# YangHai-1218/SCFlow

Hardware: AMD Instinct MI355X
Metric: image-pairs/sec at 256x256, 8 GRU iters (higher is better)
Workload: dtype f32

## Files before the change

include/scflow_hip.h:

```cpp
#ifndef SCFLOW_HIP_H
#define SCFLOW_HIP_H

#include <stdint.h>

#ifdef __cplusplus
extern "C" {
#endif

typedef void* scf_stream_t;

enum {
  SCF_OK = 0,
  SCF_EINVAL = -1,
  SCF_EUNSUPPORTED = -2,
  SCF_ELAUNCH = -3,
  SCF_ENODEVICE = -4
};

#define SCF_MAX_LEVELS 12

enum { SCF_ACT_NONE = 0, SCF_ACT_RELU = 1, SCF_ACT_SIGMOID = 2, SCF_ACT_TANH = 3 };

enum {
  SCF_CONV_PLAIN = 0,
  SCF_CONV_GRU_ZR = 1,
  SCF_CONV_GRU_Q = 2
};

#define SCF_ABI_MAJOR 5
#define SCF_VERSION (SCF_ABI_MAJOR * 100 + 3)
int scf_version(void);
const char* scf_error_string(int code);
int scf_device_count(void);

int scf_corr_build(const float* feat1, const float* feat2, float* const* levels,
                   int N, int C, int h, int w, int L, scf_stream_t stream);

int scf_corr_lookup(const float* const* levels, const float* flow, float* out,
                    int N, int h, int w, int r, int L, scf_stream_t stream);

int64_t scf_corr_level_floats(int h, int w, int level, int tiled);
unsigned scf_corr_preferred_layout(int h, int w, int r, int L);
int scf_corr_build_ex(const float* feat1, const float* feat2, float* const* levels, int N, int C,
                      int h, int w, int L, unsigned tiled_levels, scf_stream_t stream);
int scf_corr_lookup_ex(const float* const* levels, const float* flow, float* out, int N, int h,
                       int w, int r, int L, unsigned tiled_levels, scf_stream_t stream);

typedef struct scf_conv_desc {
  const float* in0; const float* in1;
  int32_t C0, C1;
  int64_t in0_nstride, in1_nstride;
  int32_t N, H, W;
  const float* wp;
  int64_t w_nstride;
  int32_t Mld;
  int32_t Cout;
  int32_t KH, KW, stride, pad_h, pad_w;
  int32_t KC;
  float* out; int64_t out_nstride;
  const float* bias;
  const float* scale; const float* shift;
  const float* res; int64_t res_nstride;
  float out_div;
  int32_t act, act2, act_split;
  int32_t mode;
  const float* gru_h; int64_t gru_h_nstride;
  float* gru_aux; int64_t gru_aux_nstride;
  const float* gru_z; int64_t gru_z_nstride;
  const void* wp_f16;
  const float* wp_a4;
  int32_t a4_groups;
  int32_t a4_mld;
  const float* wp_a4s;
  int32_t a4s_groups;
  const float* wp_thin;
  int32_t out_tile8x4;
  const float* wp_taps;
  const float* wp_a4t;
  int32_t a4t_groups;
  const float* wp_wino1d;
  const float* wp_wino;
  const float* wp_wino1d4;
  int32_t k_slices;
  int64_t out_slice_stride;
} scf_conv_desc;

int scf_conv2d(const scf_conv_desc* desc, scf_stream_t stream);

int scf_conv_workspace(scf_stream_t stream, float* ptr, int64_t floats);

int scf_conv2d_pair(const scf_conv_desc* a, const scf_conv_desc* b, scf_stream_t stream);

int64_t scf_pack_conv_weight_size(int Cout, int Cin, int KH, int KW, int KC);
int scf_pack_conv_weight(const float* w, int Cout, int Cin, int KH, int KW, int KC, float* out);
int64_t scf_pack_conv_weight_a4_size(int Cout, int Cin, int KH, int KW, int groups);
int scf_pack_conv_weight_a4(const float* w, int Cout, int Cin, int KH, int KW, int groups, float* out);
int64_t scf_pack_conv_weight_taps_size(int Cout, int Cin, int KH, int KW);
int scf_pack_conv_weight_taps(const float* w, int Cout, int Cin, int KH, int KW, float* out);
int64_t scf_pack_conv_weight_wino1d_size(int32_t Cout, int32_t Cin);
int scf_pack_conv_weight_wino1d(const float* w, int32_t Cout, int32_t Cin, float* out);
int64_t scf_pack_conv_weight_wino1d4_size(int32_t Cout, int32_t Cin);
int scf_pack_conv_weight_wino1d4(const float* w, int32_t Cout, int32_t Cin, float* out);
int64_t scf_pack_conv_weight_wino_size(int32_t Cout, int32_t Cin);
int scf_pack_conv_weight_wino(const float* w, int32_t Cout, int32_t Cin, float* out);

typedef struct scf_gru_pass {
  int32_t KH, KW, pad_h, pad_w;
  const float* wp_zr; const float* bias_zr;
  const float* wp_q; const float* bias_q;
  const float* wp_zr_a4; const float* wp_q_a4; int32_t a4_groups;
  const void* wp_zr_f16; const void* wp_q_f16;
  const float* wp_zr_k32; const float* wp_q_k32;
  const float* wp_zr_a4s; const float* wp_q_a4s; int32_t a4s_groups;
  const float* wp_zr_a4t; const float* wp_q_a4t; int32_t a4t_groups;
  const float* wp_zr_wino1d; const float* wp_q_wino1d;
  const float* wp_zr_wino1d4; const float* wp_q_wino1d4;
} scf_gru_pass;

int scf_sepconv_gru(float* hx, int64_t hx_nstride, int N, int Ch, int Cx, int H, int W,
                    const scf_gru_pass* passes, int npass, float* z, float* rh,
                    scf_stream_t stream);

int scf_sepconv_gru_ctx(float* hx, int64_t hx_nstride, int N, int Ch, int Cc, int Cx, int H, int W,
                        const scf_gru_pass* passes, int npass, const float* const* ctx,
                        int64_t ctx_nstride, float* z, float* rh, scf_stream_t stream);

typedef struct scf_iter_gn {
  const float* gamma; const float* beta; float* out;
  int32_t C, HW, G; float eps;
} scf_iter_gn;

typedef struct scf_scflow_iter {
  int32_t struct_size;
  int32_t N, H, W, h, w;
  int32_t L, radius; uint32_t tiled_levels; int32_t corr_channels;
  const float* levels[SCF_MAX_LEVELS];
  float* flow_lr;
  float* corr;
  int32_t mask_flow, mask_corr;
  const float* mask_prev;
  float* flow_masked;
  scf_conv_desc flow0, flow1, corr0, corr1, outn;
  float* flow_copy_dst;
  float* hx; int64_t hx_nstride; int32_t Ch, Cc, Cx, npass;
  scf_gru_pass gru[2];
  const float* ctx[2]; int64_t ctx_nstride;
  float* z; float* rh;
  scf_conv_desc heads, fpred, mpred, menc0, menc1, denc0, denc1;
  scf_conv_desc pose[3];
  scf_iter_gn gn[3];
  const float* fc1_w; const float* fc1_b; float* fc1_out; int32_t fc1_K, fc1_O;
  const float* fc2_w; const float* fc2_b; float* fc2_out; int32_t fc2_O;
  int32_t fc_fused, fc1_slices, fc2_slices;
  const float* rot_w; const float* rot_b; float* rot_all; int32_t rot_O;
  const float* trans_w; const float* trans_b; float* trans_all; int32_t trans_O;
  const int64_t* label; int32_t num_class, label_mode;
  const float* depth; const float* K; const float* R0; const float* t0; float invalid_flow_num;
  const float* flow_in;
  const float* R_in; const float* t_in;
  float* flow_out; float* flow_pred; float* mask_up;
  float* R_out; float* t_out; float* d_rot; float* d_trans;
  scf_stream_t side_stream; int32_t overlap_flow, overlap_mask, overlap_up;
  void* lookup_timer;
} scf_scflow_iter;

int scf_scflow_iteration(const scf_scflow_iter* iter, scf_stream_t stream);

int scf_instance_norm(const float* x, const float* res, float* out, int64_t planes,
                      int HW, float eps, int relu, scf_stream_t stream);

int scf_group_norm_relu(const float* x, const float* gamma, const float* beta, float* out,
                        int N, int C, int HW, int G, float eps, scf_stream_t stream);
int scf_group_norm_relu_parts(const float* x, int parts, int64_t part_stride, const float* gamma,
                              const float* beta, float* out, int N, int C, int HW, int G, float eps,
                              scf_stream_t stream);

int scf_linear(const float* x, const float* W, const float* b, float* y, int N, int K,
               int O, int act, scf_stream_t stream);

int scf_linear_pair(const float* x, const float* W1, const float* b1, float* y1, int O1,
                    const float* W2, const float* b2, float* y2, int O2, int N, int K, int act,
                    scf_stream_t stream);

typedef struct scf_fc_desc {
  const float* x; int32_t x_parts; int64_t x_part_stride;
  const float* x_bias; int32_t x_relu;
  int32_t gn_groups, gn_hw; const float* gn_gamma; const float* gn_beta; float gn_eps;
  int32_t N, K;
  const float* W; const float* bias; float* y; int32_t O;
  const float* W2; const float* bias2; float* y2; int32_t O2;
  int32_t act;
  int32_t slices;
} scf_fc_desc;
int scf_fc_splitk(const scf_fc_desc* desc, scf_stream_t stream);

#define SCF_POSE_LABEL_PER_SAMPLE 1
#define SCF_POSE_DEPTH_LINEAR 2
int scf_pose_update(const float* rot_all, const float* trans_all, const int64_t* label,
                    int num_class, int label_mode, const float* R_in, const float* t_in,
                    float* d_rot, float* d_trans, float* R_out, float* t_out, int N,
                    scf_stream_t stream);

int scf_reproject_flow(const float* depth, const float* K, const float* R0, const float* t0,
                       const float* R, const float* t, float* flow, int N, int H, int W,
                       float invalid_num, scf_stream_t stream);

int scf_pose_error(const double* verts, int nv, const double* gt_r, const double* gt_t,
                   const double* pred_r, const double* pred_t, const double* K,
                   const int* sample_idx, int nsel, int symmetric, double* err3d, double* err2d,
                   scf_stream_t stream);

int scf_flow_corr_2d3d(const float* flow, const float* depth, const float* occ, float occ_thresh,
                       const float* K, const float* R0, const float* t0, int N, int H, int W,
                       float* pts2d, float* pts3d, float* conf, int32_t* count, scf_stream_t stream);

enum { SCF_PNP_SAMPLE_ALL = 0, SCF_PNP_SAMPLE_TOPK = 1, SCF_PNP_SAMPLE_RANDOM = 2 };
typedef struct scf_pnp_params {
  int32_t iterations;
  float reproj_error;
  int32_t sample_mode;
  int32_t sample_num;
  uint64_t seed;
} scf_pnp_params;
int64_t scf_pnp_workspace_bytes(int N, int capacity, const scf_pnp_params* params);
int scf_pnp_ransac(const float* pts2d, const float* pts3d, const float* conf, const int32_t* count, int N,
                   int capacity, const float* K, const float* R_ref, const float* t_ref,
                   const scf_pnp_params* params, float* R, float* t, int32_t* ok, int32_t* inliers,
                   void* workspace, scf_stream_t stream);

typedef struct scf_mesh_store {
  const float* verts;
  const float* normals;
  const float* colors;
  const int32_t* faces;
  const int32_t* vert_offset;
  const int32_t* face_offset;
  int32_t num_classes;
  int32_t max_faces;
} scf_mesh_store;
typedef struct scf_render_params {
  int32_t H, W;
  int32_t default_lights;
  int32_t seperate_lights;
  float background[3];
  float norm_mean[3];
  float norm_std[3];
} scf_render_params;
double scf_render_pixel_coord(int index, int size, int other);
int64_t scf_render_workspace_bytes(int N, int max_faces);
int scf_render_mesh(const scf_mesh_store* mesh, const int32_t* labels, const float* R, const float* t,
                    const float* K, int N, const scf_render_params* params, float* zbuf, int32_t* pix_to_face,
                    float* rgba, float* rgb_nchw, void* workspace, scf_stream_t stream);

typedef struct scf_patch_params {
  double aspect_ratio;
  double size_ratio;
  double min_expand;
  int32_t out_h, out_w;
  int32_t resize;
  int32_t vertex_stride;
  int32_t keep_ratio;
  int32_t clip_border;
  int32_t fix_clip_border_quirk;
  int32_t center;
  int32_t to_rgb;
  int32_t crop_pad_val[3];
  int32_t pad_val[3];
  float mean[3];
  float std[3];
} scf_patch_params;
int64_t scf_patch_workspace_bytes(int N);
int scf_patch_boxes(const scf_mesh_store* mesh, const int32_t* labels, const float* R, const float* t,
                    const float* K, const int32_t* crop_in, int N, int frame_h, int frame_w,
                    const scf_patch_params* params, float* box, int32_t* crop, float* scale, float* transform_matrix,
                    float* k, int32_t* valid, void* workspace, scf_stream_t stream);
int scf_patch_extract(const uint8_t* frames, int F, int frame_h, int frame_w, const int32_t* frame_index, int N,
                      const void* workspace, const scf_patch_params* params, float* out, scf_stream_t stream);

int scf_filter_flow_by_mask(float* flow, const float* mask, int N, int H, int W,
                            float invalid_num, int align_corners, scf_stream_t stream);

int64_t scf_cal_epe_workspace_bytes(int N, int H, int W);
int scf_cal_epe(const float* flow_tgt, const float* flow_pred, const float* mask, int N, int H, int W,
                float max_flow, const float* threshs, int nthr, int fix_threshold_quirk, float* err_map,
                float* mean, float* ratios, float* total_mean, float* total_ratios, void* workspace,
                scf_stream_t stream);

int scf_unproject_depth(const float* depth, const float* K, const float* R0, const float* t0,
// ... 22 lines not shown
```

include/scflow_hip_prof.h:

```cpp
#ifndef SCFLOW_HIP_PROF_H
#define SCFLOW_HIP_PROF_H

#include "scflow_hip.h"

#ifdef __cplusplus
extern "C" {
#endif

typedef void* scf_timer_t;
int scf_timer_create(scf_timer_t* timer);
int scf_timer_destroy(scf_timer_t timer);
int scf_timer_elapsed_us(scf_timer_t timer, float* microseconds);
int scf_timer_arm(scf_timer_t timer);

int scf_conv2d_query(const scf_conv_desc* desc, int32_t* info);

enum {
  SCF_KERNEL_THIN = 1,
  SCF_KERNEL_TAPS = 2,
  SCF_KERNEL_WINO = 3,
  SCF_KERNEL_WINO1D = 4,
  SCF_KERNEL_F16X3 = 5,
  SCF_KERNEL_DMA = 6,
  SCF_KERNEL_MFMA = 7,
  SCF_KERNEL_MFMA_KSPLIT = 8,
  SCF_KERNEL_WINO_Q = 9,
  SCF_KERNEL_WINO1D4 = 10
};
typedef struct scf_conv_log_entry {
  int32_t kernel;
  int32_t Cin, Cout, KH, KW, stride, Ho, Wo, N;
  int32_t mode;
  int32_t paired;
  int32_t variant;
} scf_conv_log_entry;
int scf_conv_log_enable(int capacity);
enum {
  SCF_TUNE_WINO_VARIANT = 1,
  SCF_TUNE_DMA_FORCE_KSPLIT = 2,
  SCF_TUNE_DMA_KSPLIT_GROUPS = 3,
  SCF_TUNE_WINO1D4 = 4,
  SCF_TUNE_CONV_AUTOSLICE = 7,
  SCF_TUNE_LOOKUP_STORE = 6,
  SCF_TUNE_ITER_MERGE = 8,
  SCF_TUNE_WINO1D4_HALF = 9,
  SCF_TUNE_CONV_PAIR = 10,
  SCF_TUNE_LOOKUP_PIPE = 5
};
int scf_tune(int key, int value);
int scf_conv_log_read(scf_conv_log_entry* out, int max_entries);

#ifdef __cplusplus
}
#endif
#endif
```

scflow_amd/_lib.py:

```python
from __future__ import annotations

import ctypes as C
import os

_HERE = os.path.dirname(os.path.abspath(__file__))
LIB_PATH = os.path.join(_HERE, 'csrc', 'libscflow_hip.so')

SCF_OK = 0
ACT_NONE, ACT_RELU, ACT_SIGMOID, ACT_TANH = 0, 1, 2, 3
CONV_PLAIN, CONV_GRU_ZR, CONV_GRU_Q = 0, 1, 2
MAX_LEVELS = 12
ABI_MAJOR = 5

_fp = C.c_void_p


class ConvDesc(C.Structure):
    _fields_ = [
        ('in0', _fp), ('in1', _fp),
        ('C0', C.c_int32), ('C1', C.c_int32),
        ('in0_nstride', C.c_int64), ('in1_nstride', C.c_int64),
        ('N', C.c_int32), ('H', C.c_int32), ('W', C.c_int32),
        ('wp', _fp), ('w_nstride', C.c_int64),
        ('Mld', C.c_int32), ('Cout', C.c_int32),
        ('KH', C.c_int32), ('KW', C.c_int32), ('stride', C.c_int32),
        ('pad_h', C.c_int32), ('pad_w', C.c_int32), ('KC', C.c_int32),
        ('out', _fp), ('out_nstride', C.c_int64),
        ('bias', _fp), ('scale', _fp), ('shift', _fp),
        ('res', _fp), ('res_nstride', C.c_int64),
        ('out_div', C.c_float),
        ('act', C.c_int32), ('act2', C.c_int32), ('act_split', C.c_int32),
        ('mode', C.c_int32),
        ('gru_h', _fp), ('gru_h_nstride', C.c_int64),
        ('gru_aux', _fp), ('gru_aux_nstride', C.c_int64),
        ('gru_z', _fp), ('gru_z_nstride', C.c_int64),
        ('wp_f16', _fp),
        ('wp_a4', _fp),
        ('a4_groups', C.c_int32),
        ('a4_mld', C.c_int32),
        ('wp_a4s', _fp),
        ('a4s_groups', C.c_int32),
        ('wp_thin', _fp),
        ('out_tile8x4', C.c_int32),
        ('wp_taps', _fp),
        ('wp_a4t', _fp),
        ('a4t_groups', C.c_int32),
        ('wp_wino1d', _fp),
        ('wp_wino', _fp),
        ('wp_wino1d4', _fp),
        ('k_slices', C.c_int32),
        ('out_slice_stride', C.c_int64),
    ]


class GruPass(C.Structure):
    _fields_ = [
        ('KH', C.c_int32), ('KW', C.c_int32), ('pad_h', C.c_int32), ('pad_w', C.c_int32),
        ('wp_zr', _fp), ('bias_zr', _fp), ('wp_q', _fp), ('bias_q', _fp),
        ('wp_zr_a4', _fp), ('wp_q_a4', _fp), ('a4_groups', C.c_int32),
        ('wp_zr_f16', _fp), ('wp_q_f16', _fp),
        ('wp_zr_k32', _fp), ('wp_q_k32', _fp),
        ('wp_zr_a4s', _fp), ('wp_q_a4s', _fp), ('a4s_groups', C.c_int32),
        ('wp_zr_a4t', _fp), ('wp_q_a4t', _fp), ('a4t_groups', C.c_int32),
        ('wp_zr_wino1d', _fp), ('wp_q_wino1d', _fp),
        ('wp_zr_wino1d4', _fp), ('wp_q_wino1d4', _fp),
    ]


class ConvLogEntry(C.Structure):
    _fields_ = [(n, C.c_int32) for n in ('kernel', 'Cin', 'Cout', 'KH', 'KW', 'stride', 'Ho', 'Wo', 'N', 'mode', 'paired', 'variant')]


KERNEL_NAMES = {1: 'thin', 2: 'taps', 3: 'winograd', 4: 'winograd F(2,5)', 5: 'f16x3', 6: 'direct-dma',
                7: 'direct-mfma', 8: 'direct-mfma-ksplit', 9: 'winograd-q', 10: 'winograd F(4,5)'}


class FcDesc(C.Structure):
    _fields_ = [('x', _fp), ('x_parts', C.c_int32), ('x_part_stride', C.c_int64),
                ('x_bias', _fp), ('x_relu', C.c_int32),
                ('gn_groups', C.c_int32), ('gn_hw', C.c_int32), ('gn_gamma', _fp), ('gn_beta', _fp), ('gn_eps', C.c_float),
                ('N', C.c_int32), ('K', C.c_int32),
                ('W', _fp), ('bias', _fp), ('y', _fp), ('O', C.c_int32),
                ('W2', _fp), ('bias2', _fp), ('y2', _fp), ('O2', C.c_int32),
                ('act', C.c_int32), ('slices', C.c_int32)]


class PnpParams(C.Structure):
    _fields_ = [('iterations', C.c_int32), ('reproj_error', C.c_float), ('sample_mode', C.c_int32),
                ('sample_num', C.c_int32), ('seed', C.c_uint64)]


PNP_SAMPLE_ALL, PNP_SAMPLE_TOPK, PNP_SAMPLE_RANDOM = 0, 1, 2


class MeshStore(C.Structure):
    _fields_ = [('verts', _fp), ('normals', _fp), ('colors', _fp), ('faces', _fp), ('vert_offset', _fp),
                ('face_offset', _fp), ('num_classes', C.c_int32), ('max_faces', C.c_int32)]


class RenderParams(C.Structure):
    _fields_ = [('H', C.c_int32), ('W', C.c_int32), ('default_lights', C.c_int32), ('seperate_lights', C.c_int32),
                ('background', C.c_float * 3), ('norm_mean', C.c_float * 3), ('norm_std', C.c_float * 3)]


class PatchParams(C.Structure):
    _fields_ = [('aspect_ratio', C.c_double), ('size_ratio', C.c_double), ('min_expand', C.c_double),
                ('out_h', C.c_int32), ('out_w', C.c_int32), ('resize', C.c_int32), ('vertex_stride', C.c_int32),
                ('keep_ratio', C.c_int32), ('clip_border', C.c_int32), ('fix_clip_border_quirk', C.c_int32),
                ('center', C.c_int32), ('to_rgb', C.c_int32), ('crop_pad_val', C.c_int32 * 3),
                ('pad_val', C.c_int32 * 3), ('mean', C.c_float * 3), ('std', C.c_float * 3)]


class IterGN(C.Structure):
    _fields_ = [('gamma', _fp), ('beta', _fp), ('out', _fp),
                ('C', C.c_int32), ('HW', C.c_int32), ('G', C.c_int32), ('eps', C.c_float)]


class ScflowIter(C.Structure):
    _fields_ = [
        ('struct_size', C.c_int32),
        ('N', C.c_int32), ('H', C.c_int32), ('W', C.c_int32), ('h', C.c_int32), ('w', C.c_int32),
        ('L', C.c_int32), ('radius', C.c_int32), ('tiled_levels', C.c_uint32), ('corr_channels', C.c_int32),
        ('levels', _fp * MAX_LEVELS),
        ('flow_lr', _fp), ('corr', _fp),
        ('mask_flow', C.c_int32), ('mask_corr', C.c_int32), ('mask_prev', _fp), ('flow_masked', _fp),
        ('flow0', ConvDesc), ('flow1', ConvDesc), ('corr0', ConvDesc), ('corr1', ConvDesc), ('outn', ConvDesc),
        ('flow_copy_dst', _fp),
        ('hx', _fp), ('hx_nstride', C.c_int64), ('Ch', C.c_int32), ('Cc', C.c_int32), ('Cx', C.c_int32),
        ('npass', C.c_int32),
        ('gru', GruPass * 2), ('ctx', _fp * 2), ('ctx_nstride', C.c_int64), ('z', _fp), ('rh', _fp),
        ('heads', ConvDesc), ('fpred', ConvDesc), ('mpred', ConvDesc), ('menc0', ConvDesc), ('menc1', ConvDesc),
        ('denc0', ConvDesc), ('denc1', ConvDesc),
        ('pose', ConvDesc * 3), ('gn', IterGN * 3),
        ('fc1_w', _fp), ('fc1_b', _fp), ('fc1_out', _fp), ('fc1_K', C.c_int32), ('fc1_O', C.c_int32),
        ('fc2_w', _fp), ('fc2_b', _fp), ('fc2_out', _fp), ('fc2_O', C.c_int32),
        ('fc_fused', C.c_int32), ('fc1_slices', C.c_int32), ('fc2_slices', C.c_int32),
        ('rot_w', _fp), ('rot_b', _fp), ('rot_all', _fp), ('rot_O', C.c_int32),
        ('trans_w', _fp), ('trans_b', _fp), ('trans_all', _fp), ('trans_O', C.c_int32),
        ('label', _fp), ('num_class', C.c_int32), ('label_mode', C.c_int32),
        ('depth', _fp), ('K', _fp), ('R0', _fp), ('t0', _fp), ('invalid_flow_num', C.c_float),
        ('flow_in', _fp), ('R_in', _fp), ('t_in', _fp),
        ('flow_out', _fp), ('flow_pred', _fp), ('mask_up', _fp),
        ('R_out', _fp), ('t_out', _fp), ('d_rot', _fp), ('d_trans', _fp),
        ('side_stream', _fp), ('overlap_flow', C.c_int32), ('overlap_mask', C.c_int32), ('overlap_up', C.c_int32),
        ('lookup_timer', _fp),
    ]


SIGNATURES = {
    'scf_version': (C.c_int, []),
    'scf_error_string': (C.c_char_p, [C.c_int]),
    'scf_device_count': (C.c_int, []),
    'scf_corr_build': (C.c_int, [_fp, _fp, C.POINTER(_fp), C.c_int, C.c_int, C.c_int, C.c_int,
                                 C.c_int, _fp]),
    'scf_corr_lookup': (C.c_int, [C.POINTER(_fp), _fp, _fp, C.c_int, C.c_int, C.c_int, C.c_int,
                                  C.c_int, _fp]),
    'scf_corr_build_ex': (C.c_int, [_fp, _fp, C.POINTER(_fp), C.c_int, C.c_int, C.c_int, C.c_int,
                                    C.c_int, C.c_uint, _fp]),
    'scf_corr_lookup_ex': (C.c_int, [C.POINTER(_fp), _fp, _fp, C.c_int, C.c_int, C.c_int, C.c_int,
                                     C.c_int, C.c_uint, _fp]),
    'scf_corr_level_floats': (C.c_int64, [C.c_int, C.c_int, C.c_int, C.c_int]),
    'scf_corr_preferred_layout': (C.c_uint, [C.c_int, C.c_int, C.c_int, C.c_int]),
    'scf_pose_error': (C.c_int, [_fp, C.c_int, _fp, _fp, _fp, _fp, _fp, _fp, C.c_int, C.c_int, _fp, _fp, _fp]),
    'scf_filter_flow_by_mask': (C.c_int, [_fp, _fp, C.c_int, C.c_int, C.c_int, C.c_float, C.c_int, _fp]),
    'scf_cal_epe_workspace_bytes': (C.c_int64, [C.c_int, C.c_int, C.c_int]),
    'scf_cal_epe': (C.c_int, [_fp, _fp, _fp, C.c_int, C.c_int, C.c_int, C.c_float, C.POINTER(C.c_float), C.c_int, C.c_int,
                              _fp, _fp, _fp, _fp, _fp, _fp, _fp]),
    'scf_timer_create': (C.c_int, [C.POINTER(_fp)]),
    'scf_timer_destroy': (C.c_int, [_fp]),
    'scf_timer_arm': (C.c_int, [_fp]),
    'scf_timer_elapsed_us': (C.c_int, [_fp, C.POINTER(C.c_float)]),
    'scf_conv2d': (C.c_int, [C.POINTER(ConvDesc), _fp]),
    'scf_conv2d_pair': (C.c_int, [C.POINTER(ConvDesc), C.POINTER(ConvDesc), _fp]),
    'scf_conv2d_query': (C.c_int, [C.POINTER(ConvDesc), C.POINTER(C.c_int32)]),
    'scf_tune': (C.c_int, [C.c_int, C.c_int]),
    'scf_conv_log_enable': (C.c_int, [C.c_int]),
    'scf_conv_log_read': (C.c_int, [C.POINTER(ConvLogEntry), C.c_int]),
    'scf_pack_conv_weight_size': (C.c_int64, [C.c_int, C.c_int, C.c_int, C.c_int, C.c_int]),
    'scf_pack_conv_weight': (C.c_int, [_fp, C.c_int, C.c_int, C.c_int, C.c_int, C.c_int, _fp]),
    'scf_pack_conv_weight_a4_size': (C.c_int64, [C.c_int, C.c_int, C.c_int, C.c_int, C.c_int]),
    'scf_pack_conv_weight_a4': (C.c_int, [_fp, C.c_int, C.c_int, C.c_int, C.c_int, C.c_int, _fp]),
    'scf_pack_conv_weight_taps_size': (C.c_int64, [C.c_int, C.c_int, C.c_int, C.c_int]),
    'scf_pack_conv_weight_taps': (C.c_int, [_fp, C.c_int, C.c_int, C.c_int, C.c_int, _fp]),
    'scf_pack_conv_weight_wino1d_size': (C.c_int64, [C.c_int32, C.c_int32]),
    'scf_pack_conv_weight_wino1d': (C.c_int, [_fp, C.c_int32, C.c_int32, _fp]),
    'scf_pack_conv_weight_wino1d4_size': (C.c_int64, [C.c_int32, C.c_int32]),
    'scf_pack_conv_weight_wino1d4': (C.c_int, [_fp, C.c_int32, C.c_int32, _fp]),
    'scf_pack_conv_weight_wino_size': (C.c_int64, [C.c_int32, C.c_int32]),
    'scf_pack_conv_weight_wino': (C.c_int, [_fp, C.c_int32, C.c_int32, _fp]),
    'scf_sepconv_gru': (C.c_int, [_fp, C.c_int64, C.c_int, C.c_int, C.c_int, C.c_int, C.c_int,
                                  C.POINTER(GruPass), C.c_int, _fp, _fp, _fp]),
    'scf_sepconv_gru_ctx': (C.c_int, [_fp, C.c_int64, C.c_int, C.c_int, C.c_int, C.c_int, C.c_int,
                                      C.c_int, C.POINTER(GruPass), C.c_int, C.POINTER(_fp),
                                      C.c_int64, _fp, _fp, _fp]),
    'scf_scflow_iteration': (C.c_int, [C.POINTER(ScflowIter), _fp]),
    'scf_instance_norm': (C.c_int, [_fp, _fp, _fp, C.c_int64, C.c_int, C.c_float, C.c_int, _fp]),
    'scf_group_norm_relu': (C.c_int, [_fp, _fp, _fp, _fp, C.c_int, C.c_int, C.c_int, C.c_int,
                                      C.c_float, _fp]),
    'scf_conv_workspace': (C.c_int, [_fp, _fp, C.c_int64]),
    'scf_group_norm_relu_parts': (C.c_int, [_fp, C.c_int, C.c_int64, _fp, _fp, _fp, C.c_int, C.c_int, C.c_int, C.c_int,
                                            C.c_float, _fp]),
    'scf_fc_splitk': (C.c_int, [C.POINTER(FcDesc), _fp]),
    'scf_linear': (C.c_int, [_fp, _fp, _fp, _fp, C.c_int, C.c_int, C.c_int, C.c_int, _fp]),
    'scf_linear_pair': (C.c_int, [_fp, _fp, _fp, _fp, C.c_int, _fp, _fp, _fp, C.c_int, C.c_int, C.c_int,
                                  C.c_int, _fp]),
    'scf_pose_update': (C.c_int, [_fp, _fp, _fp, C.c_int, C.c_int, _fp, _fp, _fp, _fp, _fp, _fp,
                                  C.c_int, _fp]),
    'scf_reproject_flow': (C.c_int, [_fp, _fp, _fp, _fp, _fp, _fp, _fp, C.c_int, C.c_int,
                                     C.c_int, C.c_float, _fp]),
    'scf_flow_corr_2d3d': (C.c_int, [_fp, _fp, _fp, C.c_float, _fp, _fp, _fp, C.c_int, C.c_int, C.c_int,
                                     _fp, _fp, _fp, _fp, _fp]),
    'scf_pnp_workspace_bytes': (C.c_int64, [C.c_int, C.c_int, C.POINTER(PnpParams)]),
    'scf_pnp_ransac': (C.c_int, [_fp, _fp, _fp, _fp, C.c_int, C.c_int, _fp, _fp, _fp, C.POINTER(PnpParams),
                                 _fp, _fp, _fp, _fp, _fp, _fp]),
    'scf_render_pixel_coord': (C.c_double, [C.c_int, C.c_int, C.c_int]),
    'scf_render_workspace_bytes': (C.c_int64, [C.c_int, C.c_int]),
    'scf_render_mesh': (C.c_int, [C.POINTER(MeshStore), _fp, _fp, _fp, _fp, C.c_int, C.POINTER(RenderParams),
                                  _fp, _fp, _fp, _fp, _fp, _fp]),
    'scf_patch_workspace_bytes': (C.c_int64, [C.c_int]),
    'scf_patch_boxes': (C.c_int, [C.POINTER(MeshStore), _fp, _fp, _fp, _fp, _fp, C.c_int, C.c_int, C.c_int,
                                  C.POINTER(PatchParams), _fp, _fp, _fp, _fp, _fp, _fp, _fp, _fp]),
    'scf_patch_extract': (C.c_int, [_fp, C.c_int, C.c_int, C.c_int, _fp, C.c_int, _fp, C.POINTER(PatchParams), _fp,
                                    _fp]),
    'scf_unproject_depth': (C.c_int, [_fp, _fp, _fp, _fp, _fp, C.c_int, C.c_int, C.c_int, _fp]),
    'scf_resize_bilinear': (C.c_int, [_fp, _fp, _fp, C.c_int64, C.c_int, C.c_int, C.c_int,
                                      C.c_int, C.c_float, _fp]),
    'scf_convex_upsample': (C.c_int, [_fp, _fp, _fp, C.c_int, C.c_int, C.c_int, C.c_int, C.c_int,
                                      C.c_float, C.c_float, _fp]),
    'scf_avgpool2x2': (C.c_int, [_fp, _fp, C.c_int64, C.c_int, C.c_int, _fp]),
    'scf_mul_mask': (C.c_int, [_fp, C.c_int64, _fp, _fp, C.c_int64, C.c_int, C.c_int, C.c_int, _fp]),
    'scf_copy_strided': (C.c_int, [_fp, C.c_int64, _fp, C.c_int64, C.c_int, C.c_int64, _fp]),
}

_lib = None


class ScflowHipError(RuntimeError):
    pass


def load() -> C.CDLL:
    global _lib
    if _lib is not None:
        return _lib
    if not os.path.exists(LIB_PATH):
        raise ScflowHipError(
            f'{LIB_PATH} is missing: the HIP kernels are the product and there is no fallback. '
            'Build it with `python scflow_amd/csrc/build.py` (hipcc --offload-arch=gfx950).')
    lib = C.CDLL(LIB_PATH)
    lib.scf_version.restype = C.c_int
    have = lib.scf_version()
    if have // 100 != ABI_MAJOR:
        raise ScflowHipError(f'{LIB_PATH} was built with ABI major {have // 100}, this binding expects '
                             f'{ABI_MAJOR}: rebuild it (python scflow_amd/csrc/build.py --force)')
    for name, (res, args) in SIGNATURES.items():
        fn = getattr(lib, name)
        fn.restype = res
        fn.argtypes = args
    _lib = lib
    return lib


def check(code: int, what: str) -> None:
    if code != SCF_OK:
        msg = load().scf_error_string(code).decode()
        raise ScflowHipError(f'{what} failed: {msg} ({code})')
```

scflow_amd/csrc/conv_mfma.hip:

```cpp
#include <atomic>
#include <mutex>
#include <vector>
#include "scf_common.h"

typedef float f32x16 __attribute__((ext_vector_type(16)));
typedef float f32x4 __attribute__((ext_vector_type(4)));

#include "conv_kernels.h"

template <int WM, int WN, int NCP>
__device__ __forceinline__ void mfma_taps(f32x16 (&acc)[WM][WN], const float* wl, const float* pl,
                                          const int (&boff)[WN], int T, int KW, int KC, int BM,
                                          int PW, int PHW, int half, int l32) {
  for (int t = 0; t < T; ++t) {
    const int ky = t / KW, kx = t - ky * KW;
    const float* wt = wl + (t * KC + half) * BM + l32;
    const float* pt = pl + ky * PW + kx;
#pragma unroll
    for (int c = 0; c < NCP; ++c) {
      const int cp = 2 * c;
      float a[WM], b[WN];
#pragma unroll
      for (int i = 0; i < WM; ++i) a[i] = wt[cp * BM + i * 32];
#pragma unroll
// ... 508 lines not shown
  const ConvK& k = pl.k;
  const int N = d->N;
  const bool dry = r.info || r.cap;
  int32_t scratch[4];
  int32_t* info = r.info ? r.info : r.cap ? scratch : nullptr;
  hipStream_t st = scf_stream(stream);
  int out = SCF_EUNSUPPORTED;
  auto took = [&](int which, int rf) { r.which = which; out = rf; return rf != SCF_EUNSUPPORTED; };
  if (d->k_slices > 1) {
    r.which = SCF_KERNEL_DMA;
    return want_dma(d) ? scf_conv_dma_dispatch(k, N, dry, info, st, r.cap) : SCF_EUNSUPPORTED;
  }
  if (took(SCF_KERNEL_THIN, scf_conv_thin_dispatch(k, N, dry, st, r.cap))) return out;
  if (d->wp_taps && took(SCF_KERNEL_TAPS, scf_conv_taps_dispatch(k, d->wp_taps, N, dry, info, st, r.cap))) return out;
  if (d->wp_wino) {
    int quarter = 0;
    const int rw = scf_conv_wino_dispatch(k, d->wp_wino, N, dry, info, st, &quarter, r.cap);
    if (took(quarter ? SCF_KERNEL_WINO_Q : SCF_KERNEL_WINO, rw)) return out;
  }
  const int w4 = g_wino1d4.load(std::memory_order_relaxed);
  if (d->wp_wino1d4 && w4 && took(SCF_KERNEL_WINO1D4, scf_conv_wino1d4_dispatch(k, d->wp_wino1d4, N, w4 == 2, dry, info, st)))
    return out;
  if (d->wp_wino1d && took(SCF_KERNEL_WINO1D, scf_conv_wino1d_dispatch(k, d->wp_wino1d, N, dry, info, st))) return out;
  if (want_f16x3(d) && took(SCF_KERNEL_F16X3, scf_conv_f16x3_dispatch(k, N, dry, info, st))) return out;
  if (want_dma(d)) {
    float* ws = nullptr;
    int64_t ws_floats = 0;
    const bool sliced = !r.info && g_autoslice.load(std::memory_order_relaxed) && kws_lookup(st, &ws, &ws_floats);
    if (sliced && !dry) {
      const int S = scf_conv_dma_autoslice(k, N);
      const int64_t per_slice = (int64_t)N * d->Cout * k.Ho * k.Wo;
      if (S > 1 && per_slice * S <= ws_floats) {
        ConvK part = k;
        part.out = ws; part.out_ns = (long long)d->Cout * k.Ho * k.Wo;
        part.bias = nullptr; part.scale = nullptr; part.shift = nullptr; part.res = nullptr; part.res_ns = 0;
        part.out_div = 1.f; part.out_div_pow2 = 1; part.act = SCF_ACT_NONE; part.act2 = SCF_ACT_NONE; part.act_split = 0;
        part.mode = SCF_CONV_PLAIN; part.gru_h = nullptr; part.gru_aux = nullptr; part.gru_z = nullptr;
        part.kslices = S; part.slice_ns = per_slice;
        r.which = SCF_KERNEL_DMA;
        const int rs = scf_conv_dma_dispatch(part, N, false, nullptr, st);
        if (rs == SCF_OK) return scf_conv_kcombine_launch(k, ws, S, per_slice, N, st);
        if (rs != SCF_EUNSUPPORTED) return rs;
      }
    }
    if (took(SCF_KERNEL_DMA, scf_conv_dma_dispatch(k, N, dry, info, st, r.cap))) {
      if (sliced && r.cap) r.cap->variant = -1;
      return out;
    }
  }
  r.which = k.ksplit ? SCF_KERNEL_MFMA_KSPLIT : SCF_KERNEL_MFMA;
  const int WM = pl.WM, WN = pl.WN;
  if (dry) {
    if (r.info) {
      r.info[0] = WM; r.info[1] = WN; r.info[2] = (int32_t)pl.nblk;
      r.info[3] = k.T * (k.KC / 2) * WM * WN / (k.ksplit ? 4 : 1);
    }
    return SCF_OK;
  }
  const int nblk = (int)pl.nblk;
  if (k.ksplit) {
    if (k.KC == 32) return launch_ksplit<32>(k, nblk, pl.lds_bytes, st);
    if (k.KC == 8) return launch_ksplit<8>(k, nblk, pl.lds_bytes, st);
    return launch_ksplit<2>(k, nblk, pl.lds_bytes, st);
  }
#define SCF_CASE(M, Nn) if (WM == M && WN == Nn) return launch_conv<M, Nn>(k, nblk, pl.lds_bytes, st);
  SCF_CASE(1, 1) SCF_CASE(1, 2) SCF_CASE(2, 1) SCF_CASE(2, 2)
  SCF_CASE(3, 1) SCF_CASE(4, 1)
#undef SCF_CASE
  return SCF_EUNSUPPORTED;
}

namespace {
std::mutex g_log_mu;
std::vector<scf_conv_log_entry> g_log;
std::atomic<int> g_log_cap{0};
}

int scf_wino_variant_set(int v);
int scf_dma_force_ksplit_set(int v);
int scf_dma_ksplit_groups_set(int v);
int scf_lookup_pipe_set(int v);
int scf_lookup_store_set(int v);
int scf_iter_merge_set(int v);
int scf_wino1d4_half_set(int v);

extern "C" int scf_tune(int key, int value) {
  if (key == SCF_TUNE_WINO_VARIANT) return scf_wino_variant_set(value);
  if (key == SCF_TUNE_DMA_FORCE_KSPLIT) return scf_dma_force_ksplit_set(value);
  if (key == SCF_TUNE_DMA_KSPLIT_GROUPS) return scf_dma_ksplit_groups_set(value);
  if (key == SCF_TUNE_LOOKUP_PIPE) return scf_lookup_pipe_set(value);
  if (key == SCF_TUNE_LOOKUP_STORE) return scf_lookup_store_set(value);
  if (key == SCF_TUNE_ITER_MERGE) return scf_iter_merge_set(value);
  if (key == SCF_TUNE_WINO1D4_HALF) return scf_wino1d4_half_set(value);
  if (key == SCF_TUNE_CONV_AUTOSLICE) {
    if (value < 0 || value > 1) return SCF_EINVAL;
    return g_autoslice.exchange(value);
  }
  if (key == SCF_TUNE_CONV_PAIR) {
    if (value < 0 || value > 1) return SCF_EINVAL;
    return g_pair_mode.exchange(value);
  }
  if (key == SCF_TUNE_WINO1D4) {
    if (value < 0 || value > 2) return SCF_EINVAL;
    return g_wino1d4.exchange(value);
  }
  return SCF_EINVAL;
}

extern "C" int scf_conv_log_enable(int capacity) {
  std::lock_guard<std::mutex> lk(g_log_mu);
  g_log.clear();
  if (capacity > 0) g_log.reserve((size_t)capacity);
  else g_log.shrink_to_fit();
  g_log_cap.store(capacity > 0 ? capacity : 0);
  return SCF_OK;
}

extern "C" int scf_conv_log_read(scf_conv_log_entry* out, int max_entries) {
  std::lock_guard<std::mutex> lk(g_log_mu);
  const int n = (int)g_log.size();
  if (out)
    for (int i = 0; i < n && i < max_entries; ++i) out[i] = g_log[(size_t)i];
  return n;
}

static void conv_log_push(const scf_conv_desc* d, int which, int paired, int variant = -1);
extern "C" int scf_conv2d(const scf_conv_desc* d, scf_stream_t stream) {
  ConvReq r;
  const int rc = conv2d_walk(d, stream, r);
  if (rc == SCF_OK) conv_log_push(d, r.which, 0);
  return rc;
}

static void conv_log_push(const scf_conv_desc* d, int which, int paired, int variant) {
  if (g_log_cap.load(std::memory_order_relaxed) <= 0) return;
  std::lock_guard<std::mutex> lk(g_log_mu);
  if ((int)g_log.size() >= g_log_cap.load()) return;
  scf_conv_log_entry e;
  e.kernel = which; e.Cin = d->C0 + d->C1; e.Cout = d->Cout; e.KH = d->KH; e.KW = d->KW; e.stride = d->stride;
  e.Ho = (d->H + 2 * d->pad_h - d->KH) / d->stride + 1;
  e.Wo = (d->W + 2 * d->pad_w - d->KW) / d->stride + 1;
  e.N = d->N; e.mode = d->mode; e.paired = paired; e.variant = variant;
  g_log.push_back(e);
}

static bool pairable(int which, const ScfLaunchCap& c) {
  switch (which) {
    case SCF_KERNEL_THIN: return true;
    case SCF_KERNEL_TAPS: return c.variant >= 1;
    case SCF_KERNEL_WINO_Q: return c.variant >= 10 && c.variant < 20;
    case SCF_KERNEL_WINO: return c.variant >= 20;
    case SCF_KERNEL_DMA: return c.variant >= 0;
    default: return false;
  }
}

static bool capture(const scf_conv_desc* d, scf_stream_t stream, ScfLaunchCap* cap, int* which) {
  ConvReq r;
  r.cap = cap;
  const bool ok = conv2d_walk(d, stream, r) == SCF_OK && pairable(r.which, *cap);
  *which = r.which;
  return ok;
}

typedef int (*PairLaunch)(const ScfLaunchCap&, const ScfLaunchCap&, hipStream_t);

extern "C" int scf_conv2d_pair(const scf_conv_desc* a, const scf_conv_desc* b, scf_stream_t stream) {
  if (!a || !b) return SCF_EINVAL;
  ScfLaunchCap ca, cb;
  int fa = 0, fb = 0;
  if (g_pair_mode.load(std::memory_order_relaxed) != 1 && capture(a, stream, &ca, &fa) && capture(b, stream, &cb, &fb)) {
    const size_t lmax = ca.ldsb > cb.ldsb ? ca.ldsb : cb.ldsb;
    const long long slots = (long long)scf_cu_count() * (((fa == SCF_KERNEL_DMA || fb == SCF_KERNEL_DMA) && lmax > 80 * 1024) ? 1 : 2);
    const long long na = ca.nblk, nb = cb.nblk;
    auto rounds = [](long long n, long long s) { return (n + s - 1) / s; };
// ... 129 lines not shown
```

scflow_amd/csrc/norm.hip:

```cpp
#include "scf_common.h"

__device__ __forceinline__ float wave_sum(float v) {
#pragma unroll
  for (int off = 32; off > 0; off >>= 1) v += __shfl_xor(v, off);
  return v;
}

template <int NT>
__device__ __forceinline__ float block_sum(float v, float* red) {
  v = wave_sum(v);
  const int wave = threadIdx.x >> 6, lane = threadIdx.x & 63;
  __syncthreads();
  if (lane == 0) red[wave] = v;
  __syncthreads();
  float s = 0.f;
#pragma unroll
  for (int w = 0; w < NT / 64; w += 4) s += (red[w] + red[w + 1]) + (red[w + 2] + red[w + 3]);
  return s;
}

__device__ __forceinline__ float block_sum_256(float v, float* red) {
  v = wave_sum(v);
  const int wave = threadIdx.x >> 6, lane = threadIdx.x & 63;
  __syncthreads();
  if (lane == 0) red[wave] = v;
  __syncthreads();
  return (red[0] + red[1]) + (red[2] + red[3]);
}

template <int VEC4, int NT = 256>
__global__ __launch_bounds__(NT) void instance_norm_kernel(const float* x,
                                                           const float* res,
                                                           float* out, int HW,
                                                           float eps, int relu) {
  __shared__ float red[NT / 64];
  const long long pl = blockIdx.x;
  const float4* xp = reinterpret_cast<const float4*>(x + pl * HW);
  const int n4 = HW >> 2;
  float4 v[VEC4];
  float s = 0.f;
#pragma unroll
  for (int i = 0; i < VEC4; ++i) {
    const int idx = i * NT + threadIdx.x;
    v[i] = idx < n4 ? xp[idx] : make_float4(0.f, 0.f, 0.f, 0.f);
    s += (v[i].x + v[i].y) + (v[i].z + v[i].w);
  }
  const float mean = block_sum<NT>(s, red) / (float)HW;
  float q = 0.f;
#pragma unroll
  for (int i = 0; i < VEC4; ++i) {
    const int idx = i * NT + threadIdx.x;
    if (idx < n4) {
      const float a = v[i].x - mean, b = v[i].y - mean, c = v[i].z - mean, d = v[i].w - mean;
      q += (a * a + b * b) + (c * c + d * d);
    }
  }
  const float var = block_sum<NT>(q, red) / (float)HW;
  const float rstd = 1.0f / sqrtf(var + eps);
  float4* op = reinterpret_cast<float4*>(out + pl * HW);
  const float4* rp = res ? reinterpret_cast<const float4*>(res + pl * HW) : nullptr;
#pragma unroll
  for (int i = 0; i < VEC4; ++i) {
    const int idx = i * NT + threadIdx.x;
    if (idx < n4) {
      float4 o;
      o.x = (v[i].x - mean) * rstd;
      o.y = (v[i].y - mean) * rstd;
      o.z = (v[i].z - mean) * rstd;
      o.w = (v[i].w - mean) * rstd;
      if (rp) {
        const float4 r = rp[idx];
        o.x += r.x; o.y += r.y; o.z += r.z; o.w += r.w;
      }
      if (relu) {
        o.x = fmaxf(o.x, 0.f); o.y = fmaxf(o.y, 0.f); o.z = fmaxf(o.z, 0.f); o.w = fmaxf(o.w, 0.f);
      }
      scf_store4<(SCF_ST_SC1 & 2) != 0>(reinterpret_cast<float*>(op + idx), o.x, o.y, o.z, o.w);
    }
  }
}

__global__ __launch_bounds__(256) void instance_norm_generic_kernel(const float* x,
                                                                    const float* res,
                                                                    float* out, int HW,
                                                                    float eps, int relu) {
  __shared__ float red[4];
  const long long pl = blockIdx.x;
  const float* xp = x + pl * HW;
  float s = 0.f;
  for (int i = threadIdx.x; i < HW; i += 256) s += xp[i];
  const float mean = block_sum_256(s, red) / (float)HW;
  float q = 0.f;
  for (int i = threadIdx.x; i < HW; i += 256) {
    const float a = xp[i] - mean;
    q += a * a;
  }
  const float var = block_sum_256(q, red) / (float)HW;
  const float rstd = 1.0f / sqrtf(var + eps);
  for (int i = threadIdx.x; i < HW; i += 256) {
    float o = (xp[i] - mean) * rstd;
    if (res) o += res[pl * HW + i];
    if (relu) o = fmaxf(o, 0.f);
    out[pl * HW + i] = o;
  }
}

extern "C" int scf_instance_norm(const float* x, const float* res, float* out, int64_t planes,
                                 int HW, float eps, int relu, scf_stream_t stream) {
  if (!x || !out || planes <= 0 || HW <= 0) return SCF_EINVAL;
  if (planes > 0x7fffffffLL) return SCF_EUNSUPPORTED;
  hipStream_t st = scf_stream(stream);
  const dim3 grid((unsigned)planes), blk(256);
  const bool vec = (HW % 4 == 0) && ((((uintptr_t)x | (uintptr_t)out | (uintptr_t)res) & 15) == 0);
  const int n4 = HW / 4;
  if (vec && n4 <= 256) scf_launch(instance_norm_kernel<1>, grid, blk, 0, st, x, res, out, HW, eps, relu);
  else if (vec && n4 <= 1024) scf_launch(instance_norm_kernel<4>, grid, blk, 0, st, x, res, out, HW, eps, relu);
  else if (vec && n4 <= 4096) scf_launch(instance_norm_kernel<16>, grid, blk, 0, st, x, res, out, HW, eps, relu);
  else if (vec && n4 <= 8192) scf_launch((instance_norm_kernel<8, 1024>), grid, dim3(1024), 0, st, x, res, out, HW, eps, relu);
  else if (vec && n4 <= 20480) scf_launch((instance_norm_kernel<20, 1024>), grid, dim3(1024), 0, st, x, res, out, HW, eps, relu);
  else scf_launch(instance_norm_generic_kernel, grid, blk, 0, st, x, res, out, HW, eps, relu);
  return scf_launch_status();
}

__global__ __launch_bounds__(256) void group_norm_relu_kernel(const float* __restrict__ x, int parts,
                                                              long long part_stride,
                                                              const float* __restrict__ gamma,
                                                              const float* __restrict__ beta,
                                                              float* __restrict__ out, int C, int HW,
                                                              int G, float eps) {
  __shared__ float red[4];
  const int n = blockIdx.x / G, g = blockIdx.x % G;
  const int cpg = C / G;
  const int cnt = cpg * HW;
  const long long base = ((long long)n * C + (long long)g * cpg) * HW;
  const float* xp = x + base;
  auto at = [&](int i) {
    float v = xp[i];
    for (int sl = 1; sl < parts; ++sl) v += xp[(long long)sl * part_stride + i];
    return v;
  };
  constexpr int KEEP = 8;
  const bool keep = cnt <= KEEP * 256;
  float kv[KEEP];
  if (keep) {
    float u[4][KEEP];
#pragma unroll
    for (int j = 0; j < KEEP; ++j) {
      const int i = threadIdx.x + j * 256;
#pragma unroll
      for (int sl = 0; sl < 4; ++sl) u[sl][j] = (i < cnt && sl < parts) ? xp[(long long)sl * part_stride + i] : 0.f;
    }
#pragma unroll
    for (int j = 0; j < KEEP; ++j) {
      kv[j] = u[0][j];
#pragma unroll
      for (int sl = 1; sl < 4; ++sl)
        if (sl < parts) kv[j] += u[sl][j];
    }
    for (int sl = 4; sl < parts; ++sl) {
#pragma unroll
      for (int j = 0; j < KEEP; ++j) {
        const int i = threadIdx.x + j * 256;
        if (i < cnt) kv[j] += xp[(long long)sl * part_stride + i];
      }
    }
  }
  float s = 0.f;
  if (keep) {
#pragma unroll
    for (int j = 0; j < KEEP; ++j) s += kv[j];
  } else {
    for (int i = threadIdx.x; i < cnt; i += 256) s += at(i);
  }
  const float mean = block_sum_256(s, red) / (float)cnt;
  float q = 0.f;
  if (keep) {
#pragma unroll
    for (int j = 0; j < KEEP; ++j) {
      const float a = kv[j] - mean;
      q += (threadIdx.x + j * 256 < cnt) ? a * a : 0.f;
    }
  } else {
    for (int i = threadIdx.x; i < cnt; i += 256) {
      const float a = at(i) - mean;
      q += a * a;
    }
  }
  const float var = block_sum_256(q, red) / (float)cnt;
  const float rstd = 1.0f / sqrtf(var + eps);
  if (keep) {
#pragma unroll
    for (int j = 0; j < KEEP; ++j) {
      const int i = threadIdx.x + j * 256;
      if (i < cnt) {
        const int c = g * cpg + i / HW;
        out[base + i] = fmaxf((kv[j] - mean) * rstd * gamma[c] + beta[c], 0.f);
      }
    }
  } else {
    for (int i = threadIdx.x; i < cnt; i += 256) {
      const int c = g * cpg + i / HW;
      const float o = (at(i) - mean) * rstd * gamma[c] + beta[c];
      out[base + i] = fmaxf(o, 0.f);
// ... 102 lines not shown
```

scflow_amd/csrc/pose.hip:

```cpp
#include "scf_common.h"
#include "scf_pose.h"

struct PoseOut { float d_rot[6], d_trans[3], R[9], t[3]; };
struct PoseUpdateArgs {
  const float* rot_all; const float* trans_all; const long long* label; int num_class, label_mode;
  const float* R_in; const float* t_in; float* d_rot; float* d_trans; float* R_out; float* t_out;
};
__device__ __noinline__ void pose_update_one(const float* __restrict__ rot_all, const float* __restrict__ trans_all,
                                             const long long* __restrict__ label, int num_class, int label_mode,
                                             const float* R_in, const float* t_in, int n, PoseOut* o);
__device__ __forceinline__ void pose_store(const PoseOut& o, int n, float* __restrict__ d_rot, float* __restrict__ d_trans,
                                           float* R_out, float* t_out);

__global__ __launch_bounds__(256) void reproject_flow_kernel(
    const float* __restrict__ depth, const float* __restrict__ K, const float* __restrict__ R0,
    const float* __restrict__ t0, const float* R, const float* t,
    float* __restrict__ flow, int H, int W, float invalid, PoseUpdateArgs pu) {
  __shared__ PoseMats s;
  __shared__ PoseOut po;
  const int n = blockIdx.y;
  const bool fused = pu.rot_all != nullptr;
  if (fused && threadIdx.x == 224) {
    PoseOut o;
    pose_update_one(pu.rot_all, pu.trans_all, pu.label, pu.num_class, pu.label_mode, pu.R_in, pu.t_in, n, &o);
    po = o;
    if (blockIdx.x == 0) pose_store(o, n, pu.d_rot, pu.d_trans, pu.R_out, pu.t_out);
  }
  load_mats(&s, K, R0, t0, fused ? nullptr : R, fused ? nullptr : t, n);
  if (fused) {
    if (threadIdx.x < 9) s.R[threadIdx.x] = po.R[threadIdx.x];
    if (threadIdx.x >= 64 && threadIdx.x < 67) s.t[threadIdx.x - 64] = po.t[threadIdx.x - 64];
    __syncthreads();
  }
  const int hw = H * W;
  const float* dp = depth + (long long)n * hw;
  float* fx = flow + (long long)n * 2 * hw;
  float* fy = fx + hw;
  for (int idx = blockIdx.x * blockDim.x + threadIdx.x; idx < hw; idx += gridDim.x * blockDim.x) {
    const float d = dp[idx];
    float u = invalid, v = invalid;
    if (d > 0.f) {
      const int yi = idx / W, xi = idx - yi * W;
      const float x = (float)xi, y = (float)yi;
      float X, Y, Z;
      unproject(s, x, y, d, X, Y, Z);
      const float px = s.R[0] * X + s.R[1] * Y + s.R[2] * Z + s.t[0];
      const float py = s.R[3] * X + s.R[4] * Y + s.R[5] * Z + s.t[1];
      const float pz = s.R[6] * X + s.R[7] * Y + s.R[8] * Z + s.t[2];
      const float qx = s.K[0] * px + s.K[1] * py + s.K[2] * pz;
      const float qy = s.K[3] * px + s.K[4] * py + s.K[5] * pz;
      const float qz = s.K[6] * px + s.K[7] * py + s.K[8] * pz;
      u = qx / qz - x;
      v = qy / qz - y;
    }
    fx[idx] = u;
    fy[idx] = v;
  }
}

extern "C" int scf_reproject_flow(const float* depth, const float* K, const float* R0,
                                  const float* t0, const float* R, const float* t, float* flow,
                                  int N, int H, int W, float invalid_num, scf_stream_t stream) {
  if (!depth || !K || !R0 || !t0 || !R || !t || !flow || N <= 0 || H <= 0 || W <= 0) return SCF_EINVAL;
  if (N > 65535) return SCF_EUNSUPPORTED;
  const int bx = (int)(scf_cdiv((int64_t)H * W, 256) < 64 ? scf_cdiv((int64_t)H * W, 256) : 64);
  const PoseUpdateArgs none = {};
  scf_launch(reproject_flow_kernel, dim3(bx, N), dim3(256), 0, scf_stream(stream), depth, K,
                     R0, t0, R, t, flow, H, W, invalid_num, none);
  return scf_launch_status();
}

int scf_pose_update_reproject(const float* rot_all, const float* trans_all, const int64_t* label, int num_class,
                              int label_mode, const float* R_in, const float* t_in, float* d_rot, float* d_trans,
                              float* R_out, float* t_out, const float* depth, const float* K, const float* R0,
                              const float* t0, float* flow, int N, int H, int W, float invalid_num, scf_stream_t stream) {
  if (!rot_all || !trans_all || !label || !R_in || !t_in || !d_rot || !d_trans || !R_out || !t_out || num_class <= 0 ||
      (label_mode & ~(SCF_POSE_LABEL_PER_SAMPLE | SCF_POSE_DEPTH_LINEAR)))
    return SCF_EINVAL;
  if (!depth || !K || !R0 || !t0 || !flow || N <= 0 || H <= 0 || W <= 0) return SCF_EINVAL;
  if (N > 65535) return SCF_EUNSUPPORTED;
  if (R_in == R_out || t_in == t_out) return SCF_EUNSUPPORTED;
  int64_t cap = 2LL * scf_cu_count() / N;
  cap = cap < 64 ? 64 : cap;
  const int bx = (int)(scf_cdiv((int64_t)H * W, 256) < cap ? scf_cdiv((int64_t)H * W, 256) : cap);
  const PoseUpdateArgs pu = {rot_all, trans_all, (const long long*)label, num_class, label_mode, R_in, t_in,
                             d_rot, d_trans, R_out, t_out};
  scf_launch(reproject_flow_kernel, dim3(bx, N), dim3(256), 0, scf_stream(stream), depth, K,
                     R0, t0, (const float*)nullptr, (const float*)nullptr, flow, H, W, invalid_num, pu);
  return scf_launch_status();
}

__global__ __launch_bounds__(256) void unproject_depth_kernel(
    const float* __restrict__ depth, const float* __restrict__ K, const float* __restrict__ R0,
    const float* __restrict__ t0, float* __restrict__ pts, int H, int W) {
  __shared__ PoseMats s;
  const int n = blockIdx.y;
  load_mats(&s, K, R0, t0, nullptr, nullptr, n);
  const int hw = H * W;
  const float* dp = depth + (long long)n * hw;
  float* o = pts + (long long)n * 3 * hw;
  for (int idx = blockIdx.x * blockDim.x + threadIdx.x; idx < hw; idx += gridDim.x * blockDim.x) {
    const float d = dp[idx];
    float X = 0.f, Y = 0.f, Z = 0.f;
    if (d > 0.f) {
      const int yi = idx / W, xi = idx - yi * W;
      unproject(s, (float)xi, (float)yi, d, X, Y, Z);
    }
    o[idx] = X;
    o[hw + idx] = Y;
    o[2 * hw + idx] = Z;
  }
}

extern "C" int scf_unproject_depth(const float* depth, const float* K, const float* R0,
                                   const float* t0, float* pts, int N, int H, int W,
                                   scf_stream_t stream) {
  if (!depth || !K || !R0 || !t0 || !pts || N <= 0 || H <= 0 || W <= 0) return SCF_EINVAL;
  if (N > 65535) return SCF_EUNSUPPORTED;
  const int bx = (int)(scf_cdiv((int64_t)H * W, 256) < 64 ? scf_cdiv((int64_t)H * W, 256) : 64);
  scf_launch(unproject_depth_kernel, dim3(bx, N), dim3(256), 0, scf_stream(stream), depth,
                     K, R0, t0, pts, H, W);
  return scf_launch_status();
}

__device__ __noinline__ void pose_update_one(const float* __restrict__ rot_all, const float* __restrict__ trans_all,
                                             const long long* __restrict__ label, int num_class, int label_mode,
                                             const float* R_in, const float* t_in, int n, PoseOut* o) {
  long long cls = (label_mode & SCF_POSE_LABEL_PER_SAMPLE) ? label[n] : label[0];
  if (cls < 0) cls += num_class;
  if (cls < 0) cls = 0;
  if (cls >= num_class) cls = num_class - 1;
  const float* a = rot_all + ((long long)n * num_class + cls) * 6;
  const float* dt = trans_all + ((long long)n * num_class + cls) * 3;
  float o6[6], dtr[3];
  for (int i = 0; i < 6; ++i) { o6[i] = a[i]; o->d_rot[i] = o6[i]; }
  for (int i = 0; i < 3; ++i) { dtr[i] = dt[i]; o->d_trans[i] = dtr[i]; }
  float nx = sqrtf(o6[0] * o6[0] + o6[1] * o6[1] + o6[2] * o6[2]);
  nx = fmaxf(nx, 1e-12f);
  const float x0 = o6[0] / nx, x1 = o6[1] / nx, x2 = o6[2] / nx;
  float z0 = x1 * o6[5] - x2 * o6[4], z1 = x2 * o6[3] - x0 * o6[5], z2 = x0 * o6[4] - x1 * o6[3];
  float nz = fmaxf(sqrtf(z0 * z0 + z1 * z1 + z2 * z2), 1e-12f);
  z0 /= nz; z1 /= nz; z2 /= nz;
  const float y0 = z1 * x2 - z2 * x1, y1 = z2 * x0 - z0 * x2, y2 = z0 * x1 - z1 * x0;
  const float Rd[9] = {x0, y0, z0, x1, y1, z1, x2, y2, z2};
  float Rs[9], ts[3];
  for (int i = 0; i < 9; ++i) Rs[i] = R_in[n * 9 + i];
  for (int i = 0; i < 3; ++i) ts[i] = t_in[n * 3 + i];
  for (int r = 0; r < 3; ++r)
    for (int c = 0; c < 3; ++c)
      o->R[r * 3 + c] = Rd[r * 3 + 0] * Rs[0 * 3 + c] + Rd[r * 3 + 1] * Rs[1 * 3 + c] +
                        Rd[r * 3 + 2] * Rs[2 * 3 + c];
  const float vz = (label_mode & SCF_POSE_DEPTH_LINEAR) ? ts[2] * (dtr[2] + 1.f) : ts[2] / expf(dtr[2]);
  const float vx = vz * (dtr[0] / 10.f + ts[0] / ts[2]);
  const float vy = vz * (dtr[1] / 10.f + ts[1] / ts[2]);
  o->t[0] = vx;
  o->t[1] = vy;
  o->t[2] = vz;
}
__device__ __forceinline__ void pose_store(const PoseOut& o, int n, float* __restrict__ d_rot, float* __restrict__ d_trans,
                                           float* R_out, float* t_out) {
  for (int i = 0; i < 6; ++i) d_rot[n * 6 + i] = o.d_rot[i];
  for (int i = 0; i < 3; ++i) d_trans[n * 3 + i] = o.d_trans[i];
  for (int i = 0; i < 9; ++i) R_out[n * 9 + i] = o.R[i];
  for (int i = 0; i < 3; ++i) t_out[n * 3 + i] = o.t[i];
}

__global__ void pose_update_kernel(const float* __restrict__ rot_all,
                                   const float* __restrict__ trans_all,
                                   const long long* __restrict__ label, int num_class,
                                   int label_mode, const float* R_in, const float* t_in,
                                   float* __restrict__ d_rot, float* __restrict__ d_trans,
// ... 161 lines not shown
```

scflow_amd/csrc/scf_common.h:

```cpp
#pragma once
#include <hip/hip_runtime.h>
#include <hip/hip_ext.h>
#include <stdint.h>
#include <atomic>

#include "../../include/scflow_hip.h"
#include "../../include/scflow_hip_prof.h"

#define SCF_WAVE 64

static inline int scf_launch_status() {
  hipError_t e = hipGetLastError();
  return e == hipSuccess ? SCF_OK : SCF_ELAUNCH;
}

static inline hipStream_t scf_stream(scf_stream_t s) { return reinterpret_cast<hipStream_t>(s); }

static inline int64_t scf_cdiv(int64_t a, int64_t b) { return (a + b - 1) / b; }

static inline int scf_cu_count() {
  static int cus[64] = {0};
  int dev = 0;
  if (hipGetDevice(&dev) != hipSuccess || dev < 0 || dev >= 64) return 256;
  if (cus[dev] == 0) {
// ... 12 lines not shown
  if (hipFuncSetAttribute(fn, hipFuncAttributeMaxDynamicSharedMemorySize, bytes) != hipSuccess) return SCF_ELAUNCH;
  done.fetch_or(bit, std::memory_order_release);
  return SCF_OK;
}

struct ScfTimer { hipEvent_t start, stop; };
ScfTimer*& scf_armed_timer();

template <typename F, typename... Args>
static inline void scf_launch(F kernel, dim3 grid, dim3 block, size_t lds, hipStream_t st, Args... args) {
  ScfTimer*& slot = scf_armed_timer();
  if (slot) {
    ScfTimer* t = slot;
    slot = nullptr;
    hipExtLaunchKernelGGL(kernel, grid, block, (std::uint32_t)lds, st, t->start, t->stop, 0, args...);
  } else {
    hipLaunchKernelGGL(kernel, grid, block, lds, st, args...);
  }
}

__device__ __forceinline__ int scf_xcd_remap(int b, int nblk) {
  const int nx = 8;
  int q = nblk / nx, r = nblk % nx;
  int xcd = b % nx, slot = b / nx;
  int base = xcd < r ? xcd * (q + 1) : r * (q + 1) + (xcd - r) * q;
  return base + slot;
}

__device__ __forceinline__ float scf_fast_sigmoid(float v) {
  return __builtin_amdgcn_rcpf(1.f + __expf(-v));
}
__device__ __forceinline__ float scf_fast_tanh(float v) {
  const float t = __expf(-2.f * fabsf(v));
  const float r = (1.f - t) * __builtin_amdgcn_rcpf(1.f + t);
  return copysignf(r, v);
}

__device__ __forceinline__ float scf_apply_act(float v, int act) {
  switch (act) {
    case SCF_ACT_RELU: return v > 0.f ? v : 0.f;
    case SCF_ACT_SIGMOID: return 1.f / (1.f + expf(-v));
    case SCF_ACT_TANH: return tanhf(v);
    default: return v;
  }
}

#ifndef SCF_ST_SC1
#define SCF_ST_SC1 0
#endif
typedef float scf_st_f32x4 __attribute__((ext_vector_type(4)));
template <bool SC1>
__device__ __forceinline__ void scf_store4(float* p, float a, float b, float c, float d) {
  if constexpr (SC1) {
    const scf_st_f32x4 v = {a, b, c, d};
    asm volatile("global_store_dwordx4 %0, %1, off sc1\n\ts_nop 1" : : "v"(p), "v"(v) : "memory");
  } else {
    *reinterpret_cast<float4*>(p) = make_float4(a, b, c, d);
  }
}
typedef float scf_st_f32x2 __attribute__((ext_vector_type(2)));
template <bool SC1>
__device__ __forceinline__ void scf_store2(float* p, float a, float b) {
  if constexpr (SC1) {
    const scf_st_f32x2 v = {a, b};
    asm volatile("global_store_dwordx2 %0, %1, off sc1\n\ts_nop 1" : : "v"(p), "v"(v) : "memory");
  } else {
    *reinterpret_cast<scf_st_f32x2*>(p) = scf_st_f32x2{a, b};
  }
}
template <bool SC1>
__device__ __forceinline__ void scf_store1(float* p, float a) {
  if constexpr (SC1) asm volatile("global_store_dword %0, %1, off sc1" : : "v"(p), "v"(a) : "memory");
  else *p = a;
}

int scf_resize_bilinear_jobs(const float* a, const float* b, float* out, int64_t planes, float mul,
                             const float* a1, const float* b1, float* out1, int64_t planes1, float mul1,
                             float* out2, int out2_group, int64_t out2_gstride,
                             int Hin, int Win, int Hout, int Wout, scf_stream_t stream);
int scf_pose_update_reproject(const float* rot_all, const float* trans_all, const int64_t* label, int num_class,
                              int label_mode, const float* R_in, const float* t_in, float* d_rot, float* d_trans,
                              float* R_out, float* t_out, const float* depth, const float* K, const float* R0,
                              const float* t0, float* flow, int N, int H, int W, float invalid_num, scf_stream_t stream);
```

scflow_amd/csrc/scflow_iter.hip:

```cpp
#include "scf_common.h"

namespace {

struct IterEvents {
  hipEvent_t ev[7];
  bool ok = false;
  bool init() {
    if (ok) return true;
    for (int i = 0; i < 7; ++i)
      if (hipEventCreateWithFlags(&ev[i], hipEventDisableTiming) != hipSuccess) return false;
    return ok = true;
  }
};
IterEvents* iter_events() {
  static thread_local IterEvents pool[64];
  int dev = 0;
  if (hipGetDevice(&dev) != hipSuccess || dev < 0 || dev >= 64) return nullptr;
  return pool[dev].init() ? &pool[dev] : nullptr;
}

bool fork_to(hipStream_t from, hipStream_t to, hipEvent_t ev) {
  return hipEventRecord(ev, from) == hipSuccess && hipStreamWaitEvent(to, ev, 0) == hipSuccess;
}

struct OpenBranch {
  hipStream_t mainq, sideq;
  hipEvent_t join_ev;
  bool open = false;
  ~OpenBranch() {
    if (open) (void)fork_to(sideq, mainq, join_ev);
  }
};

#define SCF_TRY(call)                \
  do {                               \
    const int rc_ = (call);          \
    if (rc_ != SCF_OK) return rc_;   \
  } while (0)

}

static std::atomic<int> g_iter_merge{1};
int scf_iter_merge_set(int v) { return (v < 0 || v > 1) ? SCF_EINVAL : g_iter_merge.exchange(v); }

extern "C" int scf_scflow_iteration(const scf_scflow_iter* it, scf_stream_t stream) {
  if (!it) return SCF_EINVAL;
  const bool merge = g_iter_merge.load(std::memory_order_relaxed) != 0;
  if (it->struct_size != (int32_t)sizeof(scf_scflow_iter)) return SCF_EINVAL;
  if (!it->flow_in || !it->flow_out || !it->flow_pred || !it->mask_up || !it->flow_lr || !it->corr ||
      !it->R_in || !it->t_in || !it->R_out || !it->t_out || !it->d_rot || !it->d_trans || !it->hx ||
      it->N <= 0 || it->H <= 0 || it->W <= 0 || it->h <= 0 || it->w <= 0 || it->npass <= 0 || it->npass > 2)
    return SCF_EINVAL;
  if ((it->mask_flow || it->mask_corr) && !it->mask_prev) return SCF_EINVAL;
  const bool pair_flow = it->overlap_flow == 2, pair_mask = it->overlap_mask == 2;
  const bool any_overlap = it->overlap_flow == 1 || it->overlap_mask == 1 || it->overlap_up == 1;
  if (any_overlap && !it->side_stream) return SCF_EINVAL;
  hipStream_t mainq = scf_stream(stream), sideq = scf_stream(it->side_stream);
  IterEvents* Ep = any_overlap ? iter_events() : nullptr;
  if (any_overlap && !Ep) return SCF_ELAUNCH;
  static IterEvents none;
  IterEvents& E = Ep ? *Ep : none;
  OpenBranch br{mainq, sideq, E.ev[6]};
  const int N = it->N, hw = it->h * it->w;
  const float scale = (float)it->H / (float)it->h;

  const bool dual = merge && !it->mask_flow && it->flow_copy_dst != nullptr;
  SCF_TRY(scf_resize_bilinear_jobs(it->flow_in, nullptr, it->flow_lr, (int64_t)N * 2, 1.0f / scale, nullptr, nullptr, nullptr,
                                   0, 1.0f, dual ? it->flow_copy_dst : nullptr, 2, it->hx_nstride, it->H, it->W, it->h,
                                   it->w, stream));
  const float* flow_enc = it->flow_lr;
  if (it->mask_flow) {
    if (!it->flow_masked) return SCF_EINVAL;
    SCF_TRY(scf_mul_mask(it->flow_lr, (int64_t)2 * hw, it->mask_prev, it->flow_masked, (int64_t)2 * hw, N, 2, hw, stream));
    flow_enc = it->flow_masked;
  }
  if (it->overlap_flow == 1) {
    if (!fork_to(mainq, sideq, E.ev[0])) return SCF_ELAUNCH;
    br.open = true;
  }
  if (it->lookup_timer) scf_timer_arm(it->lookup_timer);
  const int rl = scf_corr_lookup_ex(it->levels, it->flow_lr, it->corr, N, it->h, it->w, it->radius, it->L,
                                    it->tiled_levels, stream);
  if (it->lookup_timer) scf_timer_arm(nullptr);
  SCF_TRY(rl);
  if (it->mask_corr)
    SCF_TRY(scf_mul_mask(it->corr, (int64_t)it->corr_channels * hw, it->mask_prev, it->corr,
                         (int64_t)it->corr_channels * hw, N, it->corr_channels, hw, stream));
  {
    scf_stream_t fq = it->overlap_flow == 1 ? it->side_stream : stream;
    scf_conv_desc f0 = it->flow0;
    f0.in0 = flow_enc;
    if (pair_flow) {
      SCF_TRY(scf_conv2d_pair(&it->corr0, &f0, stream));
      SCF_TRY(scf_conv2d_pair(&it->corr1, &it->flow1, stream));
    } else {
      SCF_TRY(scf_conv2d(&f0, fq));
      SCF_TRY(scf_conv2d(&it->flow1, fq));
      SCF_TRY(scf_conv2d(&it->corr0, stream));
      SCF_TRY(scf_conv2d(&it->corr1, stream));
    }
    if (it->overlap_flow == 1) {
      br.open = false;
      if (!fork_to(sideq, mainq, E.ev[1])) return SCF_ELAUNCH;
    }
    SCF_TRY(scf_conv2d(&it->outn, stream));
    if (!dual)
      SCF_TRY(scf_copy_strided(flow_enc, (int64_t)2 * hw, it->flow_copy_dst, it->hx_nstride, N, (int64_t)2 * hw, stream));
  }
  if (it->ctx[0])
    SCF_TRY(scf_sepconv_gru_ctx(it->hx, it->hx_nstride, N, it->Ch, it->Cc, it->Cx, it->h, it->w, it->gru, it->npass,
                                it->ctx, it->ctx_nstride, it->z, it->rh, stream));
  else
    SCF_TRY(scf_sepconv_gru(it->hx, it->hx_nstride, N, it->Ch, it->Cc + it->Cx, it->h, it->w, it->gru, it->npass,
                            it->z, it->rh, stream));
  SCF_TRY(scf_conv2d(&it->heads, stream));
  const bool mpred_aside = merge && it->overlap_mask == 1;
  if (mpred_aside) {
    if (!fork_to(mainq, sideq, E.ev[2])) return SCF_ELAUNCH;
    br.open = true;
  }
  if (pair_mask) {
    SCF_TRY(scf_conv2d_pair(&it->fpred, &it->mpred, stream));
  } else {
    SCF_TRY(scf_conv2d(&it->fpred, stream));
    if (!mpred_aside) SCF_TRY(scf_conv2d(&it->mpred, stream));
  }
  if (pair_mask) {
    SCF_TRY(scf_conv2d_pair(&it->denc0, &it->menc0, stream));
    SCF_TRY(scf_conv2d_pair(&it->denc1, &it->menc1, stream));
  } else {
    scf_stream_t mq = it->overlap_mask == 1 ? it->side_stream : stream;
    if (it->overlap_mask == 1 && !mpred_aside) {
      if (!fork_to(mainq, sideq, E.ev[2])) return SCF_ELAUNCH;
      br.open = true;
    }
    if (mpred_aside) SCF_TRY(scf_conv2d(&it->mpred, mq));
    SCF_TRY(scf_conv2d(&it->menc0, mq));
    SCF_TRY(scf_conv2d(&it->menc1, mq));
    SCF_TRY(scf_conv2d(&it->denc0, stream));
    SCF_TRY(scf_conv2d(&it->denc1, stream));
    if (it->overlap_mask == 1) {
      br.open = false;
      if (!fork_to(sideq, mainq, E.ev[3])) return SCF_ELAUNCH;
    }
  }
  {
    scf_stream_t uq = it->overlap_up == 1 ? it->side_stream : stream;
    if (it->overlap_up == 1) {
      if (!fork_to(mainq, sideq, E.ev[4])) return SCF_ELAUNCH;
      br.open = true;
    }
    if (!merge) {
      SCF_TRY(scf_resize_bilinear(it->flow_lr, it->fpred.out, it->flow_pred, (int64_t)N * 2, it->h, it->w, it->H, it->W,
                                  scale, uq));
      SCF_TRY(scf_resize_bilinear(it->mpred.out, nullptr, it->mask_up, (int64_t)N, it->h, it->w, it->H, it->W, 1.0f, uq));
    } else {
      SCF_TRY(scf_resize_bilinear_jobs(it->flow_lr, it->fpred.out, it->flow_pred, (int64_t)N * 2, scale, it->mpred.out, nullptr,
                                       it->mask_up, (int64_t)N, 1.0f, nullptr, 1, 0, it->h, it->w, it->H, it->W, uq));
    }
  }
  for (int i = 0; i < 3; ++i) {
    SCF_TRY(scf_conv2d(&it->pose[i], stream));
    const scf_iter_gn& g = it->gn[i];
    if (it->fc_fused && i == 2) break;
    const scf_conv_desc& pc = it->pose[i];
    SCF_TRY(scf_group_norm_relu_parts(pc.out, pc.k_slices > 1 ? pc.k_slices : 1, pc.out_slice_stride, g.gamma, g.beta, g.out,
                                      N, g.C, g.HW, g.G, g.eps, stream));
  }
  if (it->fc_fused) {
    const scf_iter_gn& g = it->gn[2];
    scf_fc_desc f = {};
    f.x = it->pose[2].out; f.x_parts = it->pose[2].k_slices > 1 ? it->pose[2].k_slices : 1;
    f.x_part_stride = it->pose[2].out_slice_stride; f.gn_groups = g.G; f.gn_hw = g.HW; f.gn_gamma = g.gamma; f.gn_beta = g.beta;
    f.gn_eps = g.eps; f.N = N; f.K = it->fc1_K; f.W = it->fc1_w; f.y = it->fc1_out; f.O = it->fc1_O; f.slices = it->fc1_slices;
    SCF_TRY(scf_fc_splitk(&f, stream));
    scf_fc_desc f2 = {};
    f2.x = it->fc1_out; f2.x_parts = it->fc1_slices; f2.x_part_stride = (int64_t)N * it->fc1_O; f2.x_bias = it->fc1_b;
    f2.x_relu = 1; f2.N = N; f2.K = it->fc1_O; f2.W = it->fc2_w; f2.y = it->fc2_out; f2.O = it->fc2_O; f2.slices = it->fc2_slices;
    SCF_TRY(scf_fc_splitk(&f2, stream));
    scf_fc_desc f3 = {};
    f3.x = it->fc2_out; f3.x_parts = it->fc2_slices; f3.x_part_stride = (int64_t)N * it->fc2_O; f3.x_bias = it->fc2_b;
    f3.x_relu = 1; f3.N = N; f3.K = it->fc2_O; f3.W = it->rot_w; f3.bias = it->rot_b; f3.y = it->rot_all; f3.O = it->rot_O;
    f3.W2 = it->trans_w; f3.bias2 = it->trans_b; f3.y2 = it->trans_all; f3.O2 = it->trans_O; f3.act = SCF_ACT_NONE; f3.slices = 1;
    SCF_TRY(scf_fc_splitk(&f3, stream));
  } else {
    SCF_TRY(scf_linear(it->gn[2].out, it->fc1_w, it->fc1_b, it->fc1_out, N, it->fc1_K, it->fc1_O, SCF_ACT_RELU, stream));
    SCF_TRY(scf_linear(it->fc1_out, it->fc2_w, it->fc2_b, it->fc2_out, N, it->fc1_O, it->fc2_O, SCF_ACT_RELU, stream));
    SCF_TRY(scf_linear_pair(it->fc2_out, it->rot_w, it->rot_b, it->rot_all, it->rot_O, it->trans_w, it->trans_b,
                            it->trans_all, it->trans_O, N, it->fc2_O, SCF_ACT_NONE, stream));
  }
  {
    const int rf = !merge ? SCF_EUNSUPPORTED : scf_pose_update_reproject(it->rot_all, it->trans_all, it->label, it->num_class, it->label_mode, it->R_in,
                                             it->t_in, it->d_rot, it->d_trans, it->R_out, it->t_out, it->depth, it->K, it->R0,
                                             it->t0, it->flow_out, N, it->H, it->W, it->invalid_flow_num, stream);
    if (rf == SCF_EUNSUPPORTED) {
      SCF_TRY(scf_pose_update(it->rot_all, it->trans_all, it->label, it->num_class, it->label_mode, it->R_in, it->t_in,
                              it->d_rot, it->d_trans, it->R_out, it->t_out, N, stream));
      SCF_TRY(scf_reproject_flow(it->depth, it->K, it->R0, it->t0, it->R_out, it->t_out, it->flow_out, N, it->H, it->W,
                                 it->invalid_flow_num, stream));
    } else {
      SCF_TRY(rf);
    }
  }
  if (it->overlap_up == 1) {
    br.open = false;
    if (!fork_to(sideq, mainq, E.ev[5])) return SCF_ELAUNCH;
  }
  return SCF_OK;
}
```

scflow_amd/modules.py:

```python
from __future__ import annotations

from typing import Dict, List, Optional, Sequence, Tuple, Union

import torch
import torch.nn as nn

from . import ops
from .ops import (ACT_NONE, ACT_RELU, ACT_SIGMOID, ACT_TANH, CONV_GRU_Q, CONV_GRU_ZR, PackedConv)
from .registry import DECODERS, ENCODERS, HEAD, build_head

Tensor = torch.Tensor

_ACTS = {None: ACT_NONE, 'ReLU': ACT_RELU, 'Sigmoid': ACT_SIGMOID, 'Tanh': ACT_TANH}


def _act_code(act_cfg: Optional[dict]) -> int:
    if act_cfg is None:
        return ACT_NONE
    kind = act_cfg.get('type')
    if kind not in _ACTS:
        raise NotImplementedError(f'activation {kind} has no HIP epilogue')
    return _ACTS[kind]


# ... 27 lines not shown
        out, stack = [], [self]
        while stack:
            m = stack.pop()
            out.append(m)
            for c in m._modules.values():
                if c is not None and not isinstance(c, HipModule):
                    stack.append(c)
        return out

    def _pack_sources(self):
        return [t for m in self._pack_modules() for d in (m._parameters, m._buffers)
                for t in d.values() if t is not None]

    def _pack_key(self):
        refs = self.__dict__.get('_pack_refs')
        if refs is None:
            if type(self)._pack_sources is not HipModule._pack_sources:
                return tuple((t.data_ptr(), t._version) for t in self._pack_sources())
            refs = self.__dict__['_pack_refs'] = [(d, n) for m in self._pack_modules()
                                                  for d in (m._parameters, m._buffers) for n in d]
        key = []
        for d, n in refs:
            t = d.get(n)
            if t is not None:
                key.append((t.data_ptr(), t._version))
        return tuple(key)

    @property
    def packed(self):
        d = self.__dict__
        key = self._pack_key()
        if d.get('_packed') is None or d.get('_packed_key') != key:
            with torch.no_grad():
                d['_packed'] = self._pack()
            d['_packed_key'] = key
        return d['_packed']


class ConvBlock(HipModule):

    def __init__(self, cin, cout, kernel_size, stride=1, padding=0, act_cfg=dict(type='ReLU'),
                 norm_cfg: Optional[dict] = None):
        super().__init__()
        self.conv = nn.Conv2d(cin, cout, kernel_size, stride=stride, padding=padding,
                              bias=norm_cfg is None)
        self.act = _act_code(act_cfg)
        self.groups = None
        if norm_cfg is not None:
            if norm_cfg.get('type') != 'GN':
                raise NotImplementedError('ConvBlock supports GN only (pose head)')
            self.groups = norm_cfg['num_groups']
            self.gn = nn.GroupNorm(self.groups, cout, eps=norm_cfg.get('eps', 1e-5))

    def _pack(self) -> PackedConv:
        c = self.conv
        return PackedConv.from_weight(c.weight, c.bias, stride=c.stride[0], padding=c.padding)

    def forward(self, x0: Tensor, x1: Optional[Tensor] = None, out: Optional[Tensor] = None) -> Tensor:
        if self.groups is None:
            return ops.conv2d(self.packed, x0, x1, out=out, act=self.act)
        if self.act != ACT_RELU:
            raise NotImplementedError('GN is fused with ReLU only')
        ks = ops.conv_kslices_for(self.packed, x0, x1)
        y = ops.conv2d(self.packed, x0, x1, kslices=ks)
        return ops.group_norm_relu(y, self.gn.weight, self.gn.bias, self.groups, self.gn.eps, out=out)


class _BasicBlock(HipModule):

    def __init__(self, inplanes, planes, stride, kind, downsample: bool):
        super().__init__()
        tag = 'in' if kind == 'IN' else 'bn'
        mk = (lambda c: nn.InstanceNorm2d(c)) if kind == 'IN' else (lambda c: nn.BatchNorm2d(c))
        self.kind, self.stride, self.tag = kind, stride, tag
        self.conv1 = nn.Conv2d(inplanes, planes, 3, stride=stride, padding=1, bias=True)
        setattr(self, tag + '1', mk(planes))
        self.conv2 = nn.Conv2d(planes, planes, 3, padding=1, bias=True)
        setattr(self, tag + '2', mk(planes))
        self.downsample = None
        if downsample:
            self.downsample = nn.Sequential(nn.Conv2d(inplanes, planes, 1, stride=stride, bias=True),
                                            mk(planes))

    def _bn(self, m):
        return (m.weight, m.bias, m.running_mean, m.running_var) if self.kind == 'BN' else None

    def _pack(self):
        n1, n2 = getattr(self, self.tag + '1'), getattr(self, self.tag + '2')
        eps = n1.eps
        p = dict(c1=PackedConv.from_weight(self.conv1.weight, self.conv1.bias, self.stride, 1,
                                           bn=self._bn(n1), eps=eps),
                 c2=PackedConv.from_weight(self.conv2.weight, self.conv2.bias, 1, 1,
                                           bn=self._bn(n2), eps=eps))
        if self.downsample is not None:
            ds = self.downsample[0]
            p['ds'] = PackedConv.from_weight(ds.weight, ds.bias, self.stride, 0,
                                             bn=self._bn(self.downsample[1]), eps=eps)
        return p

    def forward(self, x: Tensor) -> Tensor:
        p = self.packed
        if self.kind == 'BN':
            y = ops.conv2d(p['c1'], x, act=ACT_RELU)
            idt = ops.conv2d(p['ds'], x) if 'ds' in p else x
            return ops.conv2d(p['c2'], y, res=idt, act=ACT_RELU)
        y = ops.conv2d(p['c1'], x)
        ops.instance_norm(y, relu=True, out=y)
        y2 = ops.conv2d(p['c2'], y)
        if 'ds' in p:
            idt = ops.conv2d(p['ds'], x)
            ops.instance_norm(idt, out=idt)
        else:
            idt = x
        return ops.instance_norm(y2, res=idt, relu=True, out=y2)


@ENCODERS.register_module()
class RAFTEncoder(HipModule):

    def __init__(self, in_channels: int, out_channels: int, scale: float = 1 / 8,
                 net_type: str = 'Basic', norm_cfg: dict = dict(type='BN', requires_grad=True),
                 init_cfg=None, **unsupported) -> None:
        super().__init__()
        if net_type != 'Basic':
            raise NotImplementedError("only net_type='Basic' is built (SCFlow config)")
        bad = {k: v for k, v in unsupported.items()
               if v not in (None, False, -1) and k not in ('conv_cfg',)}
        if bad:
            raise NotImplementedError(f'RAFTEncoder options not built: {sorted(bad)}')
        kind = norm_cfg['type']
        if kind not in ('IN', 'BN', 'SyncBN'):
            raise NotImplementedError(f'norm {kind}')
        kind = 'IN' if kind == 'IN' else 'BN'
        self.kind, self.tag = kind, ('in' if kind == 'IN' else 'bn')
        self.in_channels, self.out_channels, self.scale = in_channels, out_channels, scale
        mk = (lambda c: nn.InstanceNorm2d(c)) if kind == 'IN' else (lambda c: nn.BatchNorm2d(c))
        self.stem_stride = 1 if scale == 1 / 4 else 2
        self.conv1 = nn.Conv2d(in_channels, 64, 7, stride=self.stem_stride, padding=3, bias=True)
        setattr(self, self.tag + '1', mk(64))
        inplanes = 64
        self.res_layers = []
        for i, (planes, stride) in enumerate(zip((64, 96, 128), (1, 2, 2)), start=1):
            layer = nn.Sequential(
                _BasicBlock(inplanes, planes, stride, kind, stride != 1 or inplanes != planes),
                _BasicBlock(planes, planes, 1, kind, False))
            self.add_module(f'res_layer{i}', layer)
            self.res_layers.append(f'res_layer{i}')
            inplanes = planes
        self.conv2 = nn.Conv2d(128, out_channels, 1)

    def _pack(self):
        n1 = getattr(self, self.tag + '1')
        bn = (n1.weight, n1.bias, n1.running_mean, n1.running_var) if self.kind == 'BN' else None
        return dict(stem=PackedConv.from_weight(self.conv1.weight, self.conv1.bias,
                                                self.stem_stride, 3, bn=bn, eps=n1.eps),
                    head=PackedConv.from_weight(self.conv2.weight, self.conv2.bias, 1, 0))

    def forward(self, x: Tensor, out: Optional[Tensor] = None, head_act: int = ACT_NONE,
                head_act2: int = ACT_NONE, head_split: int = 0) -> Tensor:
        p = self.packed
        if self.kind == 'BN':
            x = ops.conv2d(p['stem'], x, act=ACT_RELU)
        else:
            x = ops.conv2d(p['stem'], x)
            ops.instance_norm(x, relu=True, out=x)
        for name in self.res_layers:
            for blk in getattr(self, name):
                x = blk(x)
        return ops.conv2d(p['head'], x, out=out, act=head_act, act2=head_act2,
                          act_split=head_split)


def encoder_pair_supported(fe: 'RAFTEncoder', ce: 'RAFTEncoder') -> bool:
    return (fe.kind == 'IN' and ce.kind == 'BN' and fe.stem_stride == ce.stem_stride and fe.in_channels == ce.in_channels
            and fe.res_layers == ce.res_layers)


def raft_encoder_pair(fe: 'RAFTEncoder', xf: Tensor, ce: 'RAFTEncoder', xc: Tensor, out_c: Optional[Tensor] = None,
                      head_act: int = ACT_NONE, head_act2: int = ACT_NONE, head_split: int = 0) -> Tuple[Tensor, Tensor]:
    if not encoder_pair_supported(fe, ce):
        raise ValueError('raft_encoder_pair: (InstanceNorm feature encoder, BatchNorm context encoder) of one layer geometry')
    pf, pc = fe.packed, ce.packed
    yf, yc = ops.conv2d_pair((pf['stem'], xf), (pc['stem'], xc, dict(act=ACT_RELU)))
    ops.instance_norm(yf, relu=True, out=yf)
    for name in fe.res_layers:
        for bf, bc in zip(getattr(fe, name), getattr(ce, name)):
            qf, qc = bf.packed, bc.packed
            tf_, tc_ = ops.conv2d_pair((qf['c1'], yf), (qc['c1'], yc, dict(act=ACT_RELU)))
            ops.instance_norm(tf_, relu=True, out=tf_)
            if 'ds' in qf:
                if_, ic_ = ops.conv2d_pair((qf['ds'], yf), (qc['ds'], yc))
                ops.instance_norm(if_, out=if_)
            else:
                if_, ic_ = yf, yc
            uf_, yc = ops.conv2d_pair((qf['c2'], tf_), (qc['c2'], tc_, dict(res=ic_, act=ACT_RELU)))
            yf = ops.instance_norm(uf_, res=if_, relu=True, out=uf_)
    return ops.conv2d_pair((pf['head'], yf), (pc['head'], yc, dict(out=out_c, act=head_act, act2=head_act2,
                                                                  act_split=head_split)))


class CorrelationPyramid(HipModule):

    def __init__(self, num_levels: int = 4) -> None:
        super().__init__()
        self.num_levels = num_levels

    def forward(self, feat1: Tensor, feat2: Tensor, tiled_levels: int = 0) -> List[Tensor]:
        return ops.corr_build(feat1, feat2, self.num_levels, tiled_levels=tiled_levels)


class CorrLookup(HipModule):

    def __init__(self, radius: int = 4, mode: str = 'bilinear', padding_mode: str = 'zeros',
                 align_corners: bool = True) -> None:
        super().__init__()
        if mode != 'bilinear' or padding_mode != 'zeros' or not align_corners:
            raise NotImplementedError('HIP CorrLookup: bilinear / zeros / align_corners=True')
        self.r = radius

    def forward(self, corr_pyramid: Sequence[Tensor], flow: Tensor,
                tiled_levels: int = 0) -> Tensor:
        return ops.corr_lookup(corr_pyramid, flow, self.r, tiled_levels=tiled_levels)


def _pyramid_layout(feat: Tensor, radius: int, num_levels: int, allow: bool = True) -> int:
    return ops.pyramid_layout(feat.shape[-2], feat.shape[-1], radius, num_levels) if allow else 0


class MotionEncoder(HipModule):

    def __init__(self, num_levels: int = 4, radius: int = 4, net_type: str = 'Basic',
                 conv_cfg=None, norm_cfg=None, act_cfg=dict(type='ReLU')) -> None:
        super().__init__()
        if net_type not in ('Basic', 'Large') or norm_cfg is not None:
            raise NotImplementedError('MotionEncoder: Basic, no norm')
        cin = num_levels * (2 * radius + 1) ** 2
        self.corr_net = nn.Sequential(ConvBlock(cin, 256, 1, padding=0, act_cfg=act_cfg),
                                      ConvBlock(256, 192, 3, padding=1, act_cfg=act_cfg))
        self.flow_net = nn.Sequential(ConvBlock(2, 128, 7, padding=3, act_cfg=act_cfg),
                                      ConvBlock(128, 64, 3, padding=1, act_cfg=act_cfg))
        self.out_net = nn.Sequential(ConvBlock(256, 126, 3, padding=1, act_cfg=act_cfg))
        self.out_channels = [126]

    def forward(self, corr: Tensor, flow: Tensor, out: Optional[Tensor] = None,
                overlap: bool = False, cf: Optional[Tensor] = None, fork=None) -> Tensor:
        n, _, h, w = flow.shape
        dev = flow.device
        if out is None:
            out = torch.empty((n, 128, h, w), dtype=torch.float32, device=dev)
        if cf is None:
            if overlap:
                raise ValueError('overlap=True needs a cf buffer allocated before the fork point')
            cf = torch.empty((n, 256, h, w), dtype=torch.float32, device=dev)
        if not overlap and 'flow' in ops.PAIR_BRANCHES and ops._CONV_EVENTS is None:
            cn, fn = self.corr_net, self.flow_net
            c1, f1 = ops.conv2d_pair((cn[0].packed, corr, dict(act=cn[0].act)), (fn[0].packed, flow, dict(act=fn[0].act)))
            ops.conv2d_pair((cn[1].packed, c1, dict(out=cf[:, :192], act=cn[1].act)),
                            (fn[1].packed, f1, dict(out=cf[:, 192:], act=fn[1].act)))
            del c1, f1
        else:
            br = ops.side_stream(overlap, after=fork)
            with br:
                f1 = self.flow_net[0](flow)
                self.flow_net[1](f1, out=cf[:, 192:])
                del f1
            c1 = self.corr_net[0](corr)
            self.corr_net[1](c1, out=cf[:, :192])
            br.join()
        self.out_net[0](cf, out=out[:, :126])
        ops.copy_channels(flow, out[:, 126:128])
        return out


class ConvGRU(HipModule):
    _kernel = {'Conv': [3], 'SeqConv': [(1, 5), (5, 1)]}
    _padding = {'Conv': [1], 'SeqConv': [(0, 2), (2, 0)]}

    def __init__(self, h_channels: int, x_channels: int, net_type: str = 'SeqConv') -> None:
        super().__init__()
# ... 210 lines not shown
        a, b = self.flow_pred.layers[0].conv, self.mask_pred.layers[0].conv
        return PackedConv.from_weight(torch.cat([a.weight, b.weight], 0),
                                      torch.cat([a.bias, b.bias], 0), 1, 1)

    def forward(self, feat_render: Tensor, feat_real: Tensor, h_feat: Tensor, cxt_feat: Tensor,
                ref_rotation: Tensor, ref_translation: Tensor, depth: Tensor, internel_k: Tensor,
                label: Tensor, init_flow: Tensor, invalid_flow_num: float,
                _consume_state: bool = False):
        hc, cc = self.h_channels, self.cxt_channels
        n, H, W = depth.shape
        scale = 2 ** (self.num_levels - 1)
        h, w = H // scale, W // scale
        dev = depth.device
        f32 = dict(dtype=torch.float32, device=dev)

        tiled = _pyramid_layout(feat_render, self.radius, self.num_levels, self.tiled_pyramid)
        pyramid = self.corr_block(feat_render, feat_real, tiled_levels=tiled)
        hx = _as_gru_buffer(h_feat, cxt_feat, hc + cc + 128, _consume_state)
        rot, trans = ref_rotation.contiguous(), ref_translation.contiguous()
        rot0, trans0 = rot, trans
        flow = init_flow
        outs = ([], [], [], [], [], [], [])
        dm = torch.empty((n, 96, h, w), **f32)
        heads = torch.empty((n, 512, h, w), **f32)
        ctx = self.gru.context_terms(hx[:, hc:hc + cc]) if self.hoist_context else None
        ov_flow, ov_mask, ov_up = (ops.small_work(n, H, W, b) for b in ('flow', 'mask', 'upsample'))
        if self.c_iteration and ops._CONV_EVENTS is None:
            return self._forward_c(pyramid, tiled, hx, ctx, rot0, trans0, depth, internel_k, label, init_flow,
                                   invalid_flow_num, tuple(ops.branch_mode(n, H, W, b) for b in ('flow', 'mask', 'upsample')))
        mask = ops.constant((n, 1, h, w), 1.0, dev) if (self.mask_flow or self.mask_corr) else None
        cf = torch.empty((n, 256, h, w), **f32)
        zbuf = torch.empty((2, n, hc, h, w), **f32)
        for _ in range(self.iters):
            flow_lr = ops.resize_bilinear(flow, (h, w), mul=1.0 / scale)
            flow_in = ops.mul_mask(flow_lr, mask) if self.mask_flow else flow_lr
            fork = ops.fork_point() if ov_flow else None
            corr = self.corr_lookup(pyramid, flow_lr, tiled_levels=tiled)
            if self.mask_corr:
                ops.mul_mask(corr, mask, out=corr)
            self.encoder(corr, flow_in, out=hx[:, hc + cc:], overlap=ov_flow, cf=cf, fork=fork)
            hv = self.gru.forward_inplace(hx, ctx, cc, scratch=zbuf)
            ops.conv2d(self.packed, hv, out=heads, act=ACT_RELU)
            d_flow = self.flow_pred.predict(heads[:, :256])
            mask = self.mask_pred.predict(heads[:, 256:], act=ACT_SIGMOID)
            br = ops.side_stream(ov_mask)
            with br:
                m1 = self.mask_encoder[0](mask)
                self.mask_encoder[1](m1, out=dm[:, 64:])
                del m1
            d1 = self.delta_flow_encoder[0](d_flow)
            self.delta_flow_encoder[1](d1, out=dm[:, :64])
            br.join()
            flow_pred = torch.empty((n, 2, H, W), **f32)
            up_mask = torch.empty((n, 1, H, W), **f32)
            br = ops.side_stream(ov_up)
            with br:
                ops.resize_bilinear(flow_lr, (H, W), mul=float(scale), b=d_flow, out=flow_pred)
                ops.resize_bilinear(mask, (H, W), out=up_mask)
            rot_all, trans_all = self.pose_pred.features(hv, dm)
            d_rot, d_trans, rot, trans = ops.pose_update(
                rot_all, trans_all, label, self.pose_pred.num_class, rot, trans,
                self.pose_flags())
            flow = ops.reproject_flow(depth, internel_k, rot0, trans0, rot, trans,
                                      invalid_flow_num)
            br.join()
            for lst, v in zip(outs, (flow, flow_pred, rot, trans, up_mask, d_rot, d_trans)):
                lst.append(v)
        return outs


def _scflow_forward_c(self, pyramid, tiled, hx, ctx, rot0, trans0, depth, internel_k, label, init_flow,
                      invalid_flow_num, overlap):
    from ._lib import ScflowIter
    import ctypes as C
    hc, cc = self.h_channels, self.cxt_channels
    n, H, W = depth.shape
    scale = 2 ** (self.num_levels - 1)
    h, w = H // scale, W // scale
    f32 = dict(dtype=torch.float32, device=depth.device)
    iters = self.iters
    E = lambda *shape: torch.empty(shape, **f32)
    enc, ph = self.encoder, self.pose_pred
    kch = self.num_levels * (2 * self.radius + 1) ** 2
    flow_lr, flow_m, corr = E(n, 2, h, w), (E(n, 2, h, w) if self.mask_flow else None), E(n, kch, h, w)
    f1, c1, cf = E(n, 128, h, w), E(n, 256, h, w), E(n, 256, h, w)
    zbuf, heads, dm = E(2, n, hc, h, w), E(n, 512, h, w), E(n, 96, h, w)
    d_flow, mask, m1, d1 = E(n, 2, h, w), E(n, 1, h, w), E(n, 64, h, w), E(n, 128, h, w)
    ones = ops.constant((n, 1, h, w), 1.0, depth.device) if (self.mask_flow or self.mask_corr) else None
    hv, xm = hx[:, :hc], hx[:, hc + cc:]
    flows, fpreds, masks = E(iters, n, 2, H, W), E(iters, n, 2, H, W), E(iters, n, 1, H, W)
    rots, transs, drots, dtranss = E(iters, n, 3, 3), E(iters, n, 3), E(iters, n, 6), E(iters, n, 3)
    it = ScflowIter()
    it.struct_size = C.sizeof(ScflowIter)
    it.N, it.H, it.W, it.h, it.w = n, H, W, h, w
    it.L, it.radius, it.tiled_levels, it.corr_channels = len(pyramid), self.radius, int(tiled), kch
    for l, lv in enumerate(pyramid):
        it.levels[l] = lv.data_ptr()
    it.flow_lr, it.corr = flow_lr.data_ptr(), corr.data_ptr()
    it.mask_flow, it.mask_corr = int(self.mask_flow), int(self.mask_corr)
    it.flow_masked = None if flow_m is None else flow_m.data_ptr()
    keep = [pyramid, flow_lr, flow_m, corr, f1, c1, cf, zbuf, heads, dm, d_flow, mask, m1, d1, ones, hx, ctx]
    cd = lambda blk, *a, **k: ops.conv_desc(blk.packed, *a, act=blk.act, **k)[0]
    it.flow0 = cd(enc.flow_net[0], flow_lr, out=f1)
    it.flow1 = cd(enc.flow_net[1], f1, out=cf[:, 192:])
    it.corr0 = cd(enc.corr_net[0], corr, out=c1)
    it.corr1 = cd(enc.corr_net[1], c1, out=cf[:, :192])
    it.outn = cd(enc.out_net[0], cf, out=xm[:, :126])
    it.flow_copy_dst = xm[:, 126:128].data_ptr()
    it.hx, it.hx_nstride = hx.data_ptr(), hx.stride(0)
    it.Ch, it.Cc, it.Cx = hc, cc, hx.shape[1] - hc - cc
    if ctx is not None:
        packs = [(pk[1], pk[2]) for pk in self.gru._ctx_packs(cc)]
        for i, t in enumerate(ctx):
            it.ctx[i] = t.data_ptr()
        it.ctx_nstride = ctx[0].stride(0)
    else:
        packs = self.gru.packed
    arr = ops.gru_passes(packs)
    it.npass = len(packs)
    for i in range(len(packs)):
        it.gru[i] = arr[i]
    it.z, it.rh = zbuf[0].data_ptr(), zbuf[1].data_ptr()
    it.heads = ops.conv_desc(self.packed, hv, out=heads, act=ACT_RELU)[0]
    it.fpred = ops.conv_desc(self.flow_pred.packed, heads[:, :256], out=d_flow)[0]
    it.mpred = ops.conv_desc(self.mask_pred.packed, heads[:, 256:], out=mask, act=ACT_SIGMOID)[0]
    it.menc0 = cd(self.mask_encoder[0], mask, out=m1)
    it.menc1 = cd(self.mask_encoder[1], m1, out=dm[:, 64:])
    it.denc0 = cd(self.delta_flow_encoder[0], d_flow, out=d1)
    it.denc1 = cd(self.delta_flow_encoder[1], d1, out=dm[:, :64])
    x0, x1 = hv, dm
    for i, blk in enumerate(ph.conv_layers):
        if blk.groups is None or blk.act != ACT_RELU:
            raise NotImplementedError('pose head: conv + GroupNorm + ReLU blocks')
        ks = ops.conv_kslices_for(blk.packed, x0, x1)
        d_, y = ops.conv_desc(blk.packed, x0, x1, kslices=ks)
        g = torch.empty_like(y[0] if ks > 1 else y)
        it.pose[i] = d_
        it.gn[i].gamma, it.gn[i].beta, it.gn[i].out = blk.gn.weight.data_ptr(), blk.gn.bias.data_ptr(), g.data_ptr()
        it.gn[i].C, it.gn[i].HW, it.gn[i].G, it.gn[i].eps = y.shape[-3], y.shape[-2] * y.shape[-1], blk.groups, blk.gn.eps
        keep += [y, g]
        x0, x1 = g, None
    fc1, fc2 = ph.fc_layers[0][0], ph.fc_layers[1][0]
    if fc1.in_features != x0[0].numel():
        raise _lib_error(f'pose head expects {fc1.in_features} features, the maps give {x0[0].numel()}')
    s1, s2 = ph.fc_plan()
    it.fc_fused, it.fc1_slices, it.fc2_slices = int(s1 > 0), max(s1, 1), max(s2, 1)
    y1, y2 = E(max(s1, 1), n, fc1.out_features), E(max(s2, 1), n, fc2.out_features)
    ra, ta = E(n, ph.rotation_pred.out_features), E(n, ph.translation_pred.out_features)
    keep += [y1, y2, ra, ta]
    P = lambda t: None if t is None else t.data_ptr()
    it.fc1_w, it.fc1_b, it.fc1_out, it.fc1_K, it.fc1_O = P(fc1.weight), P(fc1.bias), y1.data_ptr(), fc1.in_features, fc1.out_features
    it.fc2_w, it.fc2_b, it.fc2_out, it.fc2_O = P(fc2.weight), P(fc2.bias), y2.data_ptr(), fc2.out_features
    it.rot_w, it.rot_b, it.rot_all, it.rot_O = P(ph.rotation_pred.weight), P(ph.rotation_pred.bias), ra.data_ptr(), ra.shape[1]
    it.trans_w, it.trans_b, it.trans_all, it.trans_O = (P(ph.translation_pred.weight), P(ph.translation_pred.bias),
                                                        ta.data_ptr(), ta.shape[1])
    if not label.is_cuda or label.dtype != torch.int64 or not label.is_contiguous():
        raise _lib_error('label must be a contiguous int64 GPU tensor')
    it.label, it.num_class, it.label_mode = label.data_ptr(), ph.num_class, self.pose_flags()
    for name, t in (('depth', depth), ('internel_k', internel_k), ('ref_rotation', rot0), ('ref_translation', trans0),
                    ('init_flow', init_flow)):
        ops._dense(t, name)
    it.depth, it.K, it.R0, it.t0 = depth.data_ptr(), internel_k.data_ptr(), rot0.data_ptr(), trans0.data_ptr()
    it.invalid_flow_num = float(invalid_flow_num)
    it.overlap_flow, it.overlap_mask, it.overlap_up = (int(b) for b in overlap)
    it.side_stream = ops.side_stream_handle() if any(int(b) == 1 for b in overlap) else None
    outs = ([], [], [], [], [], [], [])
    flow, rot, trans = init_flow, rot0, trans0
    for i in range(iters):
        it.flow_in, it.R_in, it.t_in = flow.data_ptr(), rot.data_ptr(), trans.data_ptr()
        it.mask_prev = None if ones is None else (ones if i == 0 else mask).data_ptr()
        flow, rot, trans = flows[i], rots[i], transs[i]
        it.flow_out, it.flow_pred, it.mask_up = flow.data_ptr(), fpreds[i].data_ptr(), masks[i].data_ptr()
        it.R_out, it.t_out, it.d_rot, it.d_trans = rot.data_ptr(), trans.data_ptr(), drots[i].data_ptr(), dtranss[i].data_ptr()
        ops.scflow_iteration(it)
        for lst, v in zip(outs, (flow, fpreds[i], rot, trans, masks[i], drots[i], dtranss[i])):
            lst.append(v)
    if any(overlap):
        pass
    del keep
    return outs


def _lib_error(msg):
    from ._lib import ScflowHipError
    return ScflowHipError(msg)


SCFlowDecoder._forward_c = _scflow_forward_c


class _RAFTDecoderBase(HipModule):
    _h_channels = {'Basic': 128, 'Small': 96}
    _cxt_channels = {'Basic': 128, 'Small': 64}

    def __init__(self, net_type: str, num_levels: int, radius: int, iters: int,
                 corr_lookup_cfg: dict = dict(type='CorrLookup', align_corners=True),
                 gru_type: str = 'SeqConv', feat_channels: Union[int, Sequence[int]] = 256,
                 mask_channels: int = 64, convex_unsample_flow: bool = True, conv_cfg=None,
                 norm_cfg=None, act_cfg=None) -> None:
        super().__init__()
        if net_type != 'Basic':
            raise NotImplementedError("RAFT decoders: net_type='Basic'")
        self.net_type, self.num_levels, self.radius, self.iters = net_type, num_levels, radius, iters
        self.h_channels = self._h_channels[net_type]
        self.cxt_channels = self._cxt_channels[net_type]
        self.mask_channels = mask_channels * (2 * radius + 1)
        self.corr_block = CorrelationPyramid(num_levels)
        cl = dict(corr_lookup_cfg)
        cl.pop('type', None)
        cl['radius'] = radius
        self.corr_lookup = CorrLookup(**cl)
        self.encoder = MotionEncoder(num_levels, radius, net_type, conv_cfg, norm_cfg, act_cfg)
        self.gru = ConvGRU(self.h_channels, 126 + 2 + self.cxt_channels, gru_type)
        self.flow_pred = XHead(self.h_channels, [256], 2, x='flow')
        self.mask_pred = XHead(self.h_channels, [256], self.mask_channels, x='mask')
        self.convex_upsample_flow = convex_unsample_flow
        self.tiled_pyramid = True
        self.hoist_context = True
        if self.mask_channels != 9 * (2 ** (num_levels - 1)) ** 2:
            raise NotImplementedError('convex up-sampling kernel: 9 x 8 x 8 mask (radius 4, 4 levels)')

    def _context(self, hx):
        hc, cc = self.h_channels, self.cxt_channels
        return self.gru.context_terms(hx[:, hc:hc + cc]) if self.hoist_context else None

    def _step(self, pyramid, flow, hx, tiled=0, ctx=None):
        hc, cc = self.h_channels, self.cxt_channels
        corr = self.corr_lookup(pyramid, flow, tiled_levels=tiled)
        self.encoder(corr, flow, out=hx[:, hc + cc:])
        hv = self.gru.forward_inplace(hx, ctx, cc)
        d_flow = self.flow_pred(hv)
        n, _, h, w = flow.shape
        return hv, ops.resize_bilinear(flow, (h, w), b=d_flow)

    def _upsample(self, x: Tensor, mask: Optional[Tensor], mul: float) -> Tensor:
        scale = 2 ** (self.num_levels - 1)
        n, c, h, w = x.shape
        if mask is None:
            return ops.resize_bilinear(x, (scale * h, scale * w), mul=mul)
        return ops.convex_upsample(x, mask, scale, x_mul=mul, mask_mul=0.25)


@DECODERS.register_module()
class RAFTDecoder(_RAFTDecoderBase):

    def forward(self, feat1: Tensor, feat2: Tensor, flow: Tensor, h_feat: Tensor,
                cxt_feat: Tensor, _consume_state: bool = False) -> List[Tensor]:
        tiled = _pyramid_layout(feat1, self.radius, self.num_levels, self.tiled_pyramid)
        pyramid = self.corr_block(feat1, feat2, tiled_levels=tiled)
        hx = _as_gru_buffer(h_feat, cxt_feat, self.h_channels + self.cxt_channels + 128,
                            _consume_state)
        scale = float(2 ** (self.num_levels - 1))
        flow = flow.contiguous()
        outs = []
        ctx = self._context(hx)
        for _ in range(self.iters):
            hv, flow = self._step(pyramid, flow, hx, tiled, ctx)
            mask = self.mask_pred(hv) if self.convex_upsample_flow else None
            outs.append(self._upsample(flow, mask, scale))
# ... 44 lines not shown
```

scflow_amd/ops.py:

```python
from __future__ import annotations

import ctypes as C
import os
import math
from dataclasses import dataclass
from typing import List, Optional, Sequence, Tuple

import torch

from . import _lib
from ._lib import (ACT_NONE, ACT_RELU, ACT_SIGMOID, ACT_TANH, CONV_GRU_Q, CONV_GRU_ZR,
                   CONV_PLAIN, ConvDesc)

Tensor = torch.Tensor

__all__ = ['record_conv_kernels', 'PackedConv', 'conv_desc', 'gru_passes', 'scflow_iteration', 'side_stream_handle', 'pyramid_layout', 'untile_level', 'level_storage_shape', 'sepconv_gru', 'pack_conv_weight', 'pack_conv_weight_f16x3', 'set_conv_precision', 'set_conv_winograd', 'get_conv_winograd', 'pack_conv_weight_wino', 'pack_conv_weight_wino1d', 'pack_conv_weight_wino1d4',
           'get_conv_precision', 'set_conv_kslices', 'conv_kslices', 'conv_kslices_for', 'constant', 'clear_constants', 'register_conv_workspace', 'choose_kc', 'conv2d', 'conv2d_pair', 'corr_build', 'corr_lookup',
           'instance_norm', 'group_norm_relu', 'linear', 'fc_splitk', 'fc_slices', 'pose_update', 'reproject_flow',
           'flow_corr_2d3d', 'pnp_params', 'pnp_ransac', 'pnp',
           'unproject_depth', 'linear_pair', 'resize_bilinear', 'convex_upsample', 'avgpool2x2', 'copy_channels',
           'ACT_NONE', 'ACT_RELU', 'ACT_SIGMOID', 'ACT_TANH', 'CONV_PLAIN', 'CONV_GRU_ZR',
           'CONV_GRU_Q']


_cur_dev = torch._C._cuda_getDevice
_raw_stream = torch._C._cuda_getCurrentRawStream


_KWS = {}
_KWS_FLOATS = 1 << 20


def register_conv_workspace(enable: bool = True) -> None:
    dev = _cur_dev()
    handle = _raw_stream(dev)
    if enable:
        ws = torch.empty((_KWS_FLOATS,), dtype=torch.float32, device=f'cuda:{dev}')
        _lib.check(_lib.load().scf_conv_workspace(handle, ws.data_ptr(), _KWS_FLOATS), 'scf_conv_workspace')
        _KWS[(dev, handle)] = ws
    elif _KWS.pop((dev, handle), None) is not None:
        _lib.check(_lib.load().scf_conv_workspace(handle, None, 0), 'scf_conv_workspace')


def _stream() -> int:
    return _raw_stream(_cur_dev())


def _dev(t: Tensor, name: str) -> None:
    if not isinstance(t, torch.Tensor) or not t.is_cuda:
        raise _lib.ScflowHipError(f'{name}: expected a tensor on the GPU (HIP path only, no CPU '
                                  'fallback)')
    if t.dtype != torch.float32:
        raise _lib.ScflowHipError(f'{name}: expected float32, got {t.dtype}')
    if t.device.index != _cur_dev():
        raise _lib.ScflowHipError(
            f'{name} lives on cuda:{t.device.index} but the current device is '
            f'cuda:{_cur_dev()}: wrap the call in torch.cuda.device(tensor.device)')


def _dense(t: Tensor, name: str) -> int:
    _dev(t, name)
    if not t.is_contiguous():
        raise _lib.ScflowHipError(f'{name}: expected a contiguous tensor')
    return t.data_ptr()


def _nchw(t: Tensor, name: str) -> Tuple[int, int, int, int, int, int]:
    _dev(t, name)
    if t.dim() != 4:
        raise _lib.ScflowHipError(f'{name}: expected 4-D NCHW')
    n, c, h, w = t.shape
    sn, sc, sh, sw = t.stride()
    ok = (sw == 1 or w == 1) and (sh == w or h == 1) and (sc == h * w or c == 1)
    if not ok:
        raise _lib.ScflowHipError(f'{name}: not a sample-strided NCHW view (strides {t.stride()})')
    if n == 1:
        sn = c * h * w
    return t.data_ptr(), n, c, h, w, sn


def _opt(t: Optional[Tensor], name: str) -> Optional[int]:
    return None if t is None else _dense(t, name)


_SIDE = {}


OVERLAP_BRANCHES = set()
OVERLAP_MAX_PIXELS = {'context': 4 * 256 * 256, 'flow': 4 * 256 * 256, 'mask': 4 * 256 * 256, 'upsample': 4 * 256 * 256}


PAIR_BRANCHES = {'context', 'flow', 'mask'}
PAIR_MAX_PIXELS = {'context': 4 * 256 * 256, 'flow': None, 'mask': None}


def branch_mode(n: int, h: int, w: int, branch: str) -> int:
    if branch in PAIR_BRANCHES:
        lim = PAIR_MAX_PIXELS.get(branch, 4 * 256 * 256)
        return 2 if lim is None or n * h * w <= lim else 0
    lim = OVERLAP_MAX_PIXELS.get(branch, 4 * 256 * 256)
    return 1 if n * h * w <= lim and branch in OVERLAP_BRANCHES else 0
# ... 501 lines not shown
            g.wp_zr_a4s, g.wp_q_a4s, g.a4s_groups = pzr.wp4s.data_ptr(), pq.wp4s.data_ptr(), pzr.g4s
        if pzr.wp4t is not None and pq.wp4t is not None and pzr.g4t == pq.g4t:
            g.wp_zr_a4t, g.wp_q_a4t, g.a4t_groups = pzr.wp4t.data_ptr(), pq.wp4t.data_ptr(), pzr.g4t
        if _CONV_WINOGRAD and not f16 and pzr.wwino1d is not None and pq.wwino1d is not None:
            g.wp_zr_wino1d, g.wp_q_wino1d = pzr.wwino1d.data_ptr(), pq.wwino1d.data_ptr()
            if pzr.wwino1d4 is not None and pq.wwino1d4 is not None:
                g.wp_zr_wino1d4, g.wp_q_wino1d4 = pzr.wwino1d4.data_ptr(), pq.wwino1d4.data_ptr()
    return arr


gru_passes = _gru_passes


def side_stream_handle() -> int:
    main = torch.cuda.current_stream()
    key = (torch.cuda.current_device(), main.cuda_stream)
    side = _SIDE.get(key)
    if side is None:
        side = _SIDE[key] = torch.cuda.Stream(device=key[0])
    return side.cuda_stream


def scflow_iteration(it: '_lib.ScflowIter') -> None:
    lib = _lib.load()
    it.lookup_timer = _LOOKUP_TIMERS.take() if _LOOKUP_TIMERS is not None else None
    _lib.check(lib.scf_scflow_iteration(C.byref(it), _stream()), 'scf_scflow_iteration')


def sepconv_gru(packs, hx: Tensor, h_channels: int, z: Tensor, rh: Tensor,
                ctx: Optional[Sequence[Tensor]] = None, ctx_channels: int = 0) -> None:
    hc = h_channels
    if ctx is not None and (ctx_channels <= 0 or len(ctx) != len(packs)):
        raise _lib.ScflowHipError('sepconv_gru: one context term per pass, ctx_channels > 0')
    if _CONV_EVENTS is not None:
        hv, xv = hx[:, :hc], hx[:, hc + ctx_channels:]
        for i, (pzr, pq) in enumerate(packs):
            if ctx is None:
                conv2d(pzr, hx, out=z, mode=CONV_GRU_ZR, gru_h=hv, gru_aux=rh)
                conv2d(pq, rh, xv, out=hv, mode=CONV_GRU_Q, gru_h=hv, gru_z=z)
            else:
                conv2d(pzr, hv, xv, out=z, mode=CONV_GRU_ZR, gru_h=hv, gru_aux=rh, res=ctx[i][:, :2 * hc])
                conv2d(pq, rh, xv, out=hv, mode=CONV_GRU_Q, gru_h=hv, gru_z=z, res=ctx[i][:, 2 * hc:])
        return
    p, n, c, h, w, sn = _nchw(hx, 'hx')
    arr = _gru_passes(packs)
    if ctx is None:
        _lib.check(_lib.load().scf_sepconv_gru(p, sn, n, hc, c - hc, h, w, arr, len(packs),
                                               _dense(z, 'z'), _dense(rh, 'rh'), _stream()),
                   'scf_sepconv_gru')
        return
    ptrs, cs = (C.c_void_p * len(ctx))(), None
    for i, t in enumerate(ctx):
        pc_, nc, cc_, hh, ww, s_ = _nchw(t, 'ctx')
        if (nc, cc_, hh, ww) != (n, 3 * hc, h, w) or (cs is not None and s_ != cs):
            raise _lib.ScflowHipError('sepconv_gru: ctx must be (N, 3*h_channels, H, W), equal strides')
        ptrs[i], cs = pc_, s_
    _lib.check(_lib.load().scf_sepconv_gru_ctx(p, sn, n, hc, ctx_channels, c - hc - ctx_channels, h, w,
                                               arr, len(packs), ptrs, cs, _dense(z, 'z'),
                                               _dense(rh, 'rh'), _stream()),
               'scf_sepconv_gru_ctx')


def _read_timers(timers):
    lib = _lib.load()
    out = []
    for tm in timers:
        us = C.c_float()
        _lib.check(lib.scf_timer_elapsed_us(tm, C.byref(us)), 'scf_timer_elapsed_us')
        lib.scf_timer_destroy(tm)
        out.append(float(us.value))
    return out


def conv_timing(enable: bool):
    global _CONV_EVENTS
    if enable:
        _CONV_EVENTS = []
        return None
    evs, _CONV_EVENTS = _CONV_EVENTS or [], None
    torch.cuda.synchronize()
    return list(zip(_read_timers([e[0] for e in evs]), [e[1] for e in evs], [e[2] for e in evs]))


TUNE_KEYS = {'wino_variant': 1, 'dma_force_ksplit': 2, 'dma_ksplit_groups': 3, 'wino1d4': 4, 'lookup_pipe': 5, 'lookup_store': 6, 'conv_autoslice': 7, 'iter_merge': 8, 'wino1d4_half': 9, 'conv_pair': 10}


def tune(key: str, value: int) -> int:
    if key not in TUNE_KEYS:
        raise ValueError(f'unknown tune key {key!r}; known: {sorted(TUNE_KEYS)}')
    prev = int(_lib.load().scf_tune(TUNE_KEYS[key], int(value)))
    if prev < 0:
        _lib.check(prev, f'scf_tune({key}, {value})')
    return prev


class record_conv_kernels:

    _active = False

    def __init__(self, capacity: int = 1 << 16) -> None:
        self.capacity, self.ran, self.paired, self.variants = capacity, [], [], []

    def __enter__(self):
        if record_conv_kernels._active:
            raise RuntimeError('record_conv_kernels does not nest (one process-wide dispatch log)')
        _lib.check(_lib.load().scf_conv_log_enable(self.capacity), 'scf_conv_log_enable')
        record_conv_kernels._active = True
        return self.ran

    def __exit__(self, *exc):
        record_conv_kernels._active = False
        lib = _lib.load()
        n = lib.scf_conv_log_read(None, 0)
        buf = (_lib.ConvLogEntry * max(n, 1))()
        n = min(lib.scf_conv_log_read(buf, n), n)
        lib.scf_conv_log_enable(0)
        for e in buf[:n]:
            self.ran.append((f'{e.Cin}->{e.Cout} {e.KH}x{e.KW}/s{e.stride} @{e.Ho}x{e.Wo} N{e.N}',
                             _lib.KERNEL_NAMES.get(e.kernel, str(e.kernel))))
            self.paired.append(e.paired)
            self.variants.append(e.variant)
        return False


def time_first_kernel(fn) -> float:
    lib = _lib.load()
    tm = C.c_void_p()
    _lib.check(lib.scf_timer_create(C.byref(tm)), 'scf_timer_create')
    lib.scf_timer_arm(tm)
    try:
        fn()
    finally:
        lib.scf_timer_arm(None)
    torch.cuda.synchronize()
    return _read_timers([tm])[0]


def pyramid_layout(h: int, w: int, radius: int = 4, num_levels: int = 4) -> int:
    return int(_lib.load().scf_corr_preferred_layout(h, w, radius, num_levels))


def level_storage_shape(h: int, w: int, level: int, tiled: bool) -> Tuple[int, int]:
    lh, lw = h >> level, w >> level
    return ((lh + 3) // 4 * 4, (lw + 7) // 8 * 8) if tiled else (lh, lw)


def untile_level(level: Tensor, lh: int, lw: int) -> Tensor:
    q, _, ph, pw = level.shape
    return (level.reshape(q, ph // 4, pw // 8, 4, 8).permute(0, 1, 3, 2, 4).reshape(q, 1, ph, pw)
            [:, :, :lh, :lw].contiguous())


def untile_level0(level0: Tensor) -> Tensor:
    return untile_level(level0, level0.shape[-2], level0.shape[-1])


def _pyramid_shapes(n: int, h: int, w: int, num_levels: int, tiled_levels: int):
    return [(n * h * w, 1, *level_storage_shape(h, w, l, bool((tiled_levels >> l) & 1)))
            for l in range(num_levels)]


def corr_build(feat1: Tensor, feat2: Tensor, num_levels: int = 4,
               out: Optional[List[Tensor]] = None, tiled_levels: int = 0) -> List[Tensor]:
    p1 = _dense(feat1, 'feat1')
    p2 = _dense(feat2, 'feat2')
    if feat1.shape != feat2.shape or feat1.dim() != 4:
        raise _lib.ScflowHipError('feat1/feat2 must be equal-shape NCHW')
# ... 67 lines not shown

    def read(self):
        lib = _lib.load()
        out = []
        for tm in self.timers[:self.used]:
            us = C.c_float()
            _lib.check(lib.scf_timer_elapsed_us(tm, C.byref(us)), 'scf_timer_elapsed_us')
            out.append(float(us.value))
        return out

    def reset(self) -> None:
        self.used = 0

    def destroy(self) -> None:
        lib = _lib.load()
        for tm in self.timers:
            lib.scf_timer_destroy(tm)
        self.timers, self.used = [], 0


_LOOKUP_TIMERS: Optional[_TimerPool] = None
_CORR_TIMERS: Optional[_TimerPool] = None


def corr_build_timing(enable: bool, reserve: int = 16):
    global _CORR_TIMERS
    if enable:
        if _CORR_TIMERS is not None:
            _CORR_TIMERS.destroy()
        _CORR_TIMERS = _TimerPool(reserve)
        return None
    pool, _CORR_TIMERS = _CORR_TIMERS, None
    if pool is None:
        return []
    torch.cuda.synchronize()
    out = pool.read()
    pool.destroy()
    return out


def corr_build_timing_reset() -> None:
    if _CORR_TIMERS is not None:
        torch.cuda.synchronize()
        _CORR_TIMERS.reset()


def corr_build_timing_read():
    if _CORR_TIMERS is None:
        return []
    torch.cuda.synchronize()
    return _CORR_TIMERS.read()


def lookup_timing(enable: bool, reserve: int = 64):
    global _LOOKUP_TIMERS
    if enable:
        if _LOOKUP_TIMERS is not None:
            _LOOKUP_TIMERS.destroy()
        _LOOKUP_TIMERS = _TimerPool(reserve)
        return None
    pool, _LOOKUP_TIMERS = _LOOKUP_TIMERS, None
    if pool is None:
        return []
    torch.cuda.synchronize()
    out = pool.read()
    pool.destroy()
    return out


def lookup_timing_reset() -> None:
    if _LOOKUP_TIMERS is not None:
        torch.cuda.synchronize()
        _LOOKUP_TIMERS.reset()


def lookup_timing_read():
    if _LOOKUP_TIMERS is None:
        return []
    torch.cuda.synchronize()
    return _LOOKUP_TIMERS.read()


def instance_norm(x: Tensor, res: Optional[Tensor] = None, relu: bool = False,
                  out: Optional[Tensor] = None, eps: float = 1e-5) -> Tensor:
    px = _dense(x, 'x')
    n, c, h, w = x.shape
    if out is None:
        out = torch.empty_like(x)
    _lib.check(_lib.load().scf_instance_norm(px, _opt(res, 'res'), _dense(out, 'out'), n * c,
                                             h * w, eps, int(relu), _stream()),
               'scf_instance_norm')
    return out


def group_norm_relu(x: Tensor, gamma: Tensor, beta: Tensor, groups: int, eps: float = 1e-5,
                    out: Optional[Tensor] = None) -> Tensor:
    px = _dense(x, 'x')
    parts, pstride = 1, 0
    if x.dim() == 5:
        parts, pstride = x.shape[0], x.stride(0)
        x = x[0]
    n, c, h, w = x.shape
    if out is None:
        out = torch.empty_like(x)
    _lib.check(_lib.load().scf_group_norm_relu_parts(px, parts, pstride, _dense(gamma, 'gamma'), _dense(beta, 'beta'),
                                                     _dense(out, 'out'), n, c, h * w, groups, eps,
                                                     _stream()), 'scf_group_norm_relu')
    return out


def linear(x: Tensor, weight: Tensor, bias: Optional[Tensor], act: int = ACT_NONE,
           out: Optional[Tensor] = None) -> Tensor:
    px = _dense(x, 'x')
    n, k = x.shape
    o = weight.shape[0]
    if weight.shape[1] != k:
        raise _lib.ScflowHipError('linear: weight/in_features mismatch')
    if out is None:
        out = torch.empty((n, o), dtype=torch.float32, device=x.device)
    _lib.check(_lib.load().scf_linear(px, _dense(weight, 'weight'), _opt(bias, 'bias'),
                                      _dense(out, 'out'), n, k, o, act, _stream()), 'scf_linear')
    return out


def fc_slices(k: int) -> int:
    if k % 8 == 0 and k <= 256:
        return 1
    return k // 256 if k % 256 == 0 else 0


def fc_splitk(x: Tensor, weight: Tensor, bias: Optional[Tensor] = None, *, x_bias: Optional[Tensor] = None,
              x_relu: bool = False, gn=None, weight2: Optional[Tensor] = None, bias2: Optional[Tensor] = None,
              act: int = ACT_NONE, slices: int = 1):
    _dev(x, 'x')
    if x.dim() == 2:
        x = x.unsqueeze(0)
    if x.dim() != 3 or not x.is_contiguous():
        raise _lib.ScflowHipError('fc_splitk: x must be a contiguous (N, K) or (parts, N, K) tensor')
    parts, n, k = x.shape
    o = weight.shape[0]
    if weight.shape[1] != k or (weight2 is not None and weight2.shape[1] != k):
        raise _lib.ScflowHipError('fc_splitk: weight / in_features mismatch')
    d = _lib.FcDesc()
    d.x, d.x_parts, d.x_part_stride = x.data_ptr(), parts, n * k
    d.x_bias, d.x_relu = _opt(x_bias, 'x_bias'), int(bool(x_relu))
    if gn is not None:
        groups, hw, gamma, beta, eps = gn
        d.gn_groups, d.gn_hw, d.gn_gamma, d.gn_beta, d.gn_eps = groups, hw, _dense(gamma, 'gamma'), _dense(beta, 'beta'), eps
    d.N, d.K = n, k
    y = torch.empty((slices, n, o) if slices > 1 else (n, o), dtype=torch.float32, device=x.device)
    d.W, d.bias, d.y, d.O = _dense(weight, 'weight'), _opt(bias, 'bias'), y.data_ptr(), o
    y2 = None
    if weight2 is not None:
        y2 = torch.empty((n, weight2.shape[0]), dtype=torch.float32, device=x.device)
        d.W2, d.bias2, d.y2, d.O2 = _dense(weight2, 'weight2'), _opt(bias2, 'bias2'), y2.data_ptr(), weight2.shape[0]
    d.act, d.slices = act, slices
    _lib.check(_lib.load().scf_fc_splitk(C.byref(d), _stream()), 'scf_fc_splitk')
    return y if y2 is None else (y, y2)


def linear_pair(x: Tensor, w1: Tensor, b1: Optional[Tensor], w2: Tensor, b2: Optional[Tensor],
                act: int = ACT_NONE) -> Tuple[Tensor, Tensor]:
    px = _dense(x, 'x')
    n, k = x.shape
    if w1.shape[1] != k or w2.shape[1] != k:
        raise _lib.ScflowHipError('linear_pair: weight/in_features mismatch')
    y1 = torch.empty((n, w1.shape[0]), dtype=torch.float32, device=x.device)
    y2 = torch.empty((n, w2.shape[0]), dtype=torch.float32, device=x.device)
    _lib.check(_lib.load().scf_linear_pair(px, _dense(w1, 'w1'), _opt(b1, 'b1'), y1.data_ptr(),
                                           w1.shape[0], _dense(w2, 'w2'), _opt(b2, 'b2'),
                                           y2.data_ptr(), w2.shape[0], n, k, act, _stream()),
               'scf_linear_pair')
    return y1, y2


def pose_update(rot_all: Tensor, trans_all: Tensor, label: Tensor, num_class: int,
                rot: Tensor, trans: Tensor, label_mode: int = 0):
    n = rot_all.shape[0]
    if not label.is_cuda or label.dtype != torch.int64 or not label.is_contiguous():
        raise _lib.ScflowHipError('label must be a contiguous int64 GPU tensor')
    dev = rot_all.device
    d_rot = torch.empty((n, 6), dtype=torch.float32, device=dev)
    d_trans = torch.empty((n, 3), dtype=torch.float32, device=dev)
    r_out = torch.empty((n, 3, 3), dtype=torch.float32, device=dev)
    t_out = torch.empty((n, 3), dtype=torch.float32, device=dev)
    _lib.check(_lib.load().scf_pose_update(
        _dense(rot_all, 'rot_all'), _dense(trans_all, 'trans_all'), label.data_ptr(), num_class,
        label_mode, _dense(rot, 'rot'), _dense(trans, 'trans'), d_rot.data_ptr(),
        d_trans.data_ptr(), r_out.data_ptr(), t_out.data_ptr(), n, _stream()), 'scf_pose_update')
    return d_rot, d_trans, r_out, t_out


def reproject_flow(depth: Tensor, k: Tensor, rot0: Tensor, trans0: Tensor, rot: Tensor,
                   trans: Tensor, invalid_num: float = 0., out: Optional[Tensor] = None) -> Tensor:
    n, h, w = depth.shape
    if out is None:
        out = torch.empty((n, 2, h, w), dtype=torch.float32, device=depth.device)
    _lib.check(_lib.load().scf_reproject_flow(
        _dense(depth, 'depth'), _dense(k, 'k'), _dense(rot0, 'rot0'), _dense(trans0, 'trans0'),
        _dense(rot, 'rot'), _dense(trans, 'trans'), _dense(out, 'out'), n, h, w,
        float(invalid_num), _stream()), 'scf_reproject_flow')
    return out


def filter_flow_by_mask_(flow: Tensor, mask: Tensor, invalid_num: float = 400.,
                         align_corners: bool = False) -> Tensor:
    n, two, h, w = flow.shape
    if two != 2 or tuple(mask.shape) != (n, h, w):
        raise _lib.ScflowHipError('filter_flow_by_mask: flow (N,2,H,W), mask (N,H,W)')
    _lib.check(_lib.load().scf_filter_flow_by_mask(_dense(flow, 'flow'), _dense(mask, 'mask'), n, h, w,
                                                   float(invalid_num), int(align_corners), _stream()),
               'scf_filter_flow_by_mask')
    return flow


def _mats(t: Tensor, n: int, shape: Tuple[int, ...], name: str) -> int:
    if tuple(t.shape) != (n, *shape):
        raise _lib.ScflowHipError(f'{name}: expected shape {(n, *shape)}, got {tuple(t.shape)}')
    return _dense(t, name)


def flow_corr_2d3d(flow: Tensor, depth: Tensor, k: Tensor, rot0: Tensor, trans0: Tensor,
                   occlusion: Optional[Tensor] = None, occ_thresh: float = 0.5):
    if depth.dim() != 3:
        raise _lib.ScflowHipError('flow_corr_2d3d: depth must be (N,H,W)')
    n, h, w = depth.shape
    if tuple(flow.shape) != (n, 2, h, w):
        raise _lib.ScflowHipError(f'flow_corr_2d3d: flow must be {(n, 2, h, w)}, got {tuple(flow.shape)}')
    if occlusion is not None and tuple(occlusion.shape) != (n, h, w):
        raise _lib.ScflowHipError(f'flow_corr_2d3d: occlusion must be {(n, h, w)}, got {tuple(occlusion.shape)}')
    dev = depth.device
    pts2d = torch.empty((n, h * w, 2), dtype=torch.float32, device=dev)
    pts3d = torch.empty((n, h * w, 3), dtype=torch.float32, device=dev)
    conf = torch.empty((n, h * w), dtype=torch.float32, device=dev)
    count = torch.empty((n,), dtype=torch.int32, device=dev)
    _lib.check(_lib.load().scf_flow_corr_2d3d(
        _dense(flow, 'flow'), _dense(depth, 'depth'), _opt(occlusion, 'occlusion'), float(occ_thresh),
        _mats(k, n, (3, 3), 'k'), _mats(rot0, n, (3, 3), 'rot0'), _mats(trans0, n, (3,), 'trans0'), n, h, w,
        pts2d.data_ptr(), pts3d.data_ptr(), conf.data_ptr(), count.data_ptr(), _stream()), 'scf_flow_corr_2d3d')
    return pts2d, pts3d, conf, count


_PNP_MODES = {None: _lib.PNP_SAMPLE_ALL, 'topk': _lib.PNP_SAMPLE_TOPK, 'random': _lib.PNP_SAMPLE_RANDOM}


def pnp_params(iterations: int = 100, reproj_error: float = 3.0, sample_mode: Optional[str] = None,
               sample_num: int = 1000, seed: int = 0) -> '_lib.PnpParams':
    if isinstance(iterations, bool) or int(iterations) != iterations or iterations <= 0:
        raise _lib.ScflowHipError(f'pnp: iterations must be a positive integer, got {iterations!r}')
    if not math.isfinite(float(reproj_error)) or float(reproj_error) < 0:
        raise _lib.ScflowHipError(f'pnp: reproj_error must be finite and >= 0, got {reproj_error!r}')
    if sample_mode not in _PNP_MODES:
        raise _lib.ScflowHipError(f"pnp: sample_mode must be None, 'topk' or 'random', got {sample_mode!r}")
    if sample_mode is not None and (int(sample_num) != sample_num or sample_num <= 0):
        raise _lib.ScflowHipError(f'pnp: sample_num must be a positive integer, got {sample_num!r}')
    if int(seed) != seed or not 0 <= seed < 2 ** 64:
        raise _lib.ScflowHipError(f'pnp: seed must be an integer in [0, 2^64), got {seed!r}')
    return _lib.PnpParams(int(iterations), float(reproj_error), _PNP_MODES[sample_mode],
                          int(sample_num) if sample_mode is not None else 0, int(seed))


def pnp_ransac(pts2d: Tensor, pts3d: Tensor, count: Tensor, k: Tensor, ref_rot: Tensor, ref_trans: Tensor,
               conf: Optional[Tensor] = None, iterations: int = 100, reproj_error: float = 3.0,
               sample_mode: Optional[str] = None, sample_num: int = 1000, seed: int = 0):
    p = pnp_params(iterations, reproj_error, sample_mode, sample_num, seed)
    if pts2d.dim() != 3 or pts2d.shape[2] != 2:
        raise _lib.ScflowHipError('pnp_ransac: pts2d must be (N,C,2)')
    n, cap = pts2d.shape[0], pts2d.shape[1]
    if tuple(pts3d.shape) != (n, cap, 3):
        raise _lib.ScflowHipError(f'pnp_ransac: pts3d must be {(n, cap, 3)}, got {tuple(pts3d.shape)}')
    if conf is not None and tuple(conf.shape) != (n, cap):
        raise _lib.ScflowHipError(f'pnp_ransac: conf must be {(n, cap)}, got {tuple(conf.shape)}')
    if sample_mode == 'topk' and conf is None:
        raise _lib.ScflowHipError("pnp_ransac: sample_mode='topk' needs conf")
    if (not isinstance(count, torch.Tensor) or not count.is_cuda or count.dtype != torch.int32
            or tuple(count.shape) != (n,) or not count.is_contiguous() or count.device != pts2d.device):
        raise _lib.ScflowHipError(f'pnp_ransac: count must be a contiguous int32 GPU tensor of shape {(n,)}')
    if n == 0 or cap == 0:
        raise _lib.ScflowHipError('pnp_ransac: empty batch')
    lib = _lib.load()
    dev = pts2d.device
    wsb = lib.scf_pnp_workspace_bytes(n, cap, C.byref(p))
    _lib.check(min(int(wsb), 0), 'scf_pnp_workspace_bytes')
    ws = torch.empty((max(int(wsb), 1),), dtype=torch.uint8, device=dev) if wsb > 0 else None
    rot = torch.empty((n, 3, 3), dtype=torch.float32, device=dev)
# ... 252 lines not shown
```

Baseline: 2312.

## Defer per-iteration full-res outputs to one batched pass after GRU loop

Adds a deferred-output mode where each iteration only computes the pose update and the next low-resolution reprojected flow (fused into one kernel). The full-resolution reprojected flows, upsampled flow predictions and masks for all iterations are then produced in one batched scflow_outputs launch after the loop. This is meant to remove per-iteration full-res kernels from the serial critical path and cut launch count. It also adds an instance-norm variant that normalizes the residual in the same kernel. The cost is per-iteration buffers for d_flow, mask and flow_lr, plus ABI changes.

```diff
diff --git a/include/scflow_hip.h b/include/scflow_hip.h
--- a/include/scflow_hip.h
+++ b/include/scflow_hip.h
@@ -27,7 +27,7 @@
   SCF_CONV_GRU_Q = 2
 };
 
-#define SCF_ABI_MAJOR 5
+#define SCF_ABI_MAJOR 6
 #define SCF_VERSION (SCF_ABI_MAJOR * 100 + 3)
 int scf_version(void);
 const char* scf_error_string(int code);
@@ -162,12 +162,21 @@
   float* R_out; float* t_out; float* d_rot; float* d_trans;
   scf_stream_t side_stream; int32_t overlap_flow, overlap_mask, overlap_up;
   void* lookup_timer;
+  int32_t defer_outputs, flow_lr_ready;
+  float* flow_lr_next;
 } scf_scflow_iter;
 
 int scf_scflow_iteration(const scf_scflow_iter* iter, scf_stream_t stream);
+
+int scf_scflow_outputs(const float* depth, const float* K, const float* R0, const float* t0, const float* rots,
+                       const float* transs, float* flows, const float* flow_lr, const float* d_flow,
+                       const float* mask_lr, float* fpreds, float* masks, int iters, int N, int H, int W, int h, int w,
+                       float invalid_flow_num, scf_stream_t stream);
 
 int scf_instance_norm(const float* x, const float* res, float* out, int64_t planes,
                       int HW, float eps, int relu, scf_stream_t stream);
+int scf_instance_norm_ex(const float* x, float* res, float* out, int64_t planes, int HW, float eps, int relu,
+                         int res_norm, scf_stream_t stream);
 
 int scf_group_norm_relu(const float* x, const float* gamma, const float* beta, float* out,
                         int N, int C, int HW, int G, float eps, scf_stream_t stream);
@@ -204,6 +213,12 @@
 int scf_reproject_flow(const float* depth, const float* K, const float* R0, const float* t0,
                        const float* R, const float* t, float* flow, int N, int H, int W,
                        float invalid_num, scf_stream_t stream);
+
+int scf_pose_update_flow_lr(const float* rot_all, const float* trans_all, const int64_t* label, int num_class,
+                            int label_mode, const float* R_in, const float* t_in, float* d_rot, float* d_trans,
+                            float* R_out, float* t_out, const float* depth, const float* K, const float* R0,
+                            const float* t0, float* flow_lr, float* flow_copy, int64_t flow_copy_nstride, int N,
+                            int H, int W, int h, int w, float mul, float invalid_num, scf_stream_t stream);
 
 int scf_pose_error(const double* verts, int nv, const double* gt_r, const double* gt_t,
                    const double* pred_r, const double* pred_t, const double* K,
diff --git a/include/scflow_hip_prof.h b/include/scflow_hip_prof.h
--- a/include/scflow_hip_prof.h
+++ b/include/scflow_hip_prof.h
@@ -43,6 +43,7 @@
   SCF_TUNE_CONV_AUTOSLICE = 7,
   SCF_TUNE_LOOKUP_STORE = 6,
   SCF_TUNE_ITER_MERGE = 8,
+  SCF_TUNE_ITER_DEFER = 11,
   SCF_TUNE_WINO1D4_HALF = 9,
   SCF_TUNE_CONV_PAIR = 10,
   SCF_TUNE_LOOKUP_PIPE = 5
diff --git a/scflow_amd/_lib.py b/scflow_amd/_lib.py
--- a/scflow_amd/_lib.py
+++ b/scflow_amd/_lib.py
@@ -10,7 +10,7 @@
 ACT_NONE, ACT_RELU, ACT_SIGMOID, ACT_TANH = 0, 1, 2, 3
 CONV_PLAIN, CONV_GRU_ZR, CONV_GRU_Q = 0, 1, 2
 MAX_LEVELS = 12
-ABI_MAJOR = 5
+ABI_MAJOR = 6
 
 _fp = C.c_void_p
 
@@ -144,6 +144,7 @@
         ('R_out', _fp), ('t_out', _fp), ('d_rot', _fp), ('d_trans', _fp),
         ('side_stream', _fp), ('overlap_flow', C.c_int32), ('overlap_mask', C.c_int32), ('overlap_up', C.c_int32),
         ('lookup_timer', _fp),
+        ('defer_outputs', C.c_int32), ('flow_lr_ready', C.c_int32), ('flow_lr_next', _fp),
     ]
 
 
@@ -195,6 +196,12 @@
                                       C.c_int64, _fp, _fp, _fp]),
     'scf_scflow_iteration': (C.c_int, [C.POINTER(ScflowIter), _fp]),
     'scf_instance_norm': (C.c_int, [_fp, _fp, _fp, C.c_int64, C.c_int, C.c_float, C.c_int, _fp]),
+    'scf_instance_norm_ex': (C.c_int, [_fp, _fp, _fp, C.c_int64, C.c_int, C.c_float, C.c_int, C.c_int, _fp]),
+    'scf_scflow_outputs': (C.c_int, [_fp, _fp, _fp, _fp, _fp, _fp, _fp, _fp, _fp, _fp, _fp, _fp, C.c_int, C.c_int, C.c_int,
+                                     C.c_int, C.c_int, C.c_int, C.c_float, _fp]),
+    'scf_pose_update_flow_lr': (C.c_int, [_fp, _fp, _fp, C.c_int, C.c_int, _fp, _fp, _fp, _fp, _fp, _fp, _fp, _fp, _fp, _fp,
+                                          _fp, _fp, C.c_int64, C.c_int, C.c_int, C.c_int, C.c_int, C.c_int, C.c_float,
+                                          C.c_float, _fp]),
     'scf_group_norm_relu': (C.c_int, [_fp, _fp, _fp, _fp, C.c_int, C.c_int, C.c_int, C.c_int,
                                       C.c_float, _fp]),
     'scf_conv_workspace': (C.c_int, [_fp, _fp, C.c_int64]),
diff --git a/scflow_amd/csrc/conv_mfma.hip b/scflow_amd/csrc/conv_mfma.hip
--- a/scflow_amd/csrc/conv_mfma.hip
+++ b/scflow_amd/csrc/conv_mfma.hip
@@ -614,6 +614,7 @@
 int scf_lookup_pipe_set(int v);
 int scf_lookup_store_set(int v);
 int scf_iter_merge_set(int v);
+int scf_iter_defer_set(int v);
 int scf_wino1d4_half_set(int v);
 
 extern "C" int scf_tune(int key, int value) {
@@ -623,6 +624,7 @@
   if (key == SCF_TUNE_LOOKUP_PIPE) return scf_lookup_pipe_set(value);
   if (key == SCF_TUNE_LOOKUP_STORE) return scf_lookup_store_set(value);
   if (key == SCF_TUNE_ITER_MERGE) return scf_iter_merge_set(value);
+  if (key == SCF_TUNE_ITER_DEFER) return scf_iter_defer_set(value);
   if (key == SCF_TUNE_WINO1D4_HALF) return scf_wino1d4_half_set(value);
   if (key == SCF_TUNE_CONV_AUTOSLICE) {
     if (value < 0 || value > 1) return SCF_EINVAL;
diff --git a/scflow_amd/csrc/norm.hip b/scflow_amd/csrc/norm.hip
--- a/scflow_amd/csrc/norm.hip
+++ b/scflow_amd/csrc/norm.hip
@@ -28,7 +28,7 @@
   return (red[0] + red[1]) + (red[2] + red[3]);
 }
 
-template <int VEC4, int NT = 256>
+template <int VEC4, int NT = 256, bool RN = false>
 __global__ __launch_bounds__(NT) void instance_norm_kernel(const float* x,
                                                            const float* res,
                                                            float* out, int HW,
@@ -59,6 +59,36 @@
   const float rstd = 1.0f / sqrtf(var + eps);
   float4* op = reinterpret_cast<float4*>(out + pl * HW);
   const float4* rp = res ? reinterpret_cast<const float4*>(res + pl * HW) : nullptr;
+  float4 rv[RN ? VEC4 : 1];
+  if constexpr (RN) {
+    float rs = 0.f;
+#pragma unroll
+    for (int i = 0; i < VEC4; ++i) {
+      const int idx = i * NT + threadIdx.x;
+      rv[i] = idx < n4 ? rp[idx] : make_float4(0.f, 0.f, 0.f, 0.f);
+      rs += (rv[i].x + rv[i].y) + (rv[i].z + rv[i].w);
+    }
+    const float rmean = block_sum<NT>(rs, red) / (float)HW;
+    float rq = 0.f;
+#pragma unroll
+    for (int i = 0; i < VEC4; ++i) {
+      const int idx = i * NT + threadIdx.x;
+      if (idx < n4) {
+        const float a = rv[i].x - rmean, b = rv[i].y - rmean, c = rv[i].z - rmean, d = rv[i].w - rmean;
+        rq += (a * a + b * b) + (c * c + d * d);
+      }
+    }
+    const float rvar = block_sum<NT>(rq, red) / (float)HW;
+    const float rrstd = 1.0f / sqrtf(rvar + eps);
+#pragma unroll
+    for (int i = 0; i < VEC4; ++i) {
+#pragma clang fp contract(off)
+      rv[i].x = (rv[i].x - rmean) * rrstd;
+      rv[i].y = (rv[i].y - rmean) * rrstd;
+      rv[i].z = (rv[i].z - rmean) * rrstd;
+      rv[i].w = (rv[i].w - rmean) * rrstd;
+    }
+  }
 #pragma unroll
   for (int i = 0; i < VEC4; ++i) {
     const int idx = i * NT + threadIdx.x;
@@ -69,7 +99,9 @@
       o.z = (v[i].z - mean) * rstd;
       o.w = (v[i].w - mean) * rstd;
       if (rp) {
-        const float4 r = rp[idx];
+        float4 r;
+        if constexpr (RN) r = rv[i];
+        else r = rp[idx];
         o.x += r.x; o.y += r.y; o.z += r.z; o.w += r.w;
       }
       if (relu) {
@@ -80,6 +112,7 @@
   }
 }
 
+template <bool RN = false>
 __global__ __launch_bounds__(256) void instance_norm_generic_kernel(const float* x,
                                                                     const float* res,
                                                                     float* out, int HW,
@@ -97,9 +130,29 @@
   }
   const float var = block_sum_256(q, red) / (float)HW;
   const float rstd = 1.0f / sqrtf(var + eps);
+  float rmean = 0.f, rrstd = 0.f;
+  if constexpr (RN) {
+    const float* rp = res + pl * HW;
+    float rs = 0.f;
+    for (int i = threadIdx.x; i < HW; i += 256) rs += rp[i];
+    rmean = block_sum_256(rs, red) / (float)HW;
+    float rq = 0.f;
+    for (int i = threadIdx.x; i < HW; i += 256) {
+      const float a = rp[i] - rmean;
+      rq += a * a;
+    }
+    rrstd = 1.0f / sqrtf(block_sum_256(rq, red) / (float)HW + eps);
+  }
   for (int i = threadIdx.x; i < HW; i += 256) {
     float o = (xp[i] - mean) * rstd;
-    if (res) o += res[pl * HW + i];
+    if (res) {
+      float r = res[pl * HW + i];
+      if constexpr (RN) {
+#pragma clang fp contract(off)
+        r = (r - rmean) * rrstd;
+      }
+      o += r;
+    }
     if (relu) o = fmaxf(o, 0.f);
     out[pl * HW + i] = o;
   }
@@ -118,7 +171,28 @@
   else if (vec && n4 <= 4096) scf_launch(instance_norm_kernel<16>, grid, blk, 0, st, x, res, out, HW, eps, relu);
   else if (vec && n4 <= 8192) scf_launch((instance_norm_kernel<8, 1024>), grid, dim3(1024), 0, st, x, res, out, HW, eps, relu);
   else if (vec && n4 <= 20480) scf_launch((instance_norm_kernel<20, 1024>), grid, dim3(1024), 0, st, x, res, out, HW, eps, relu);
-  else scf_launch(instance_norm_generic_kernel, grid, blk, 0, st, x, res, out, HW, eps, relu);
+  else scf_launch(instance_norm_generic_kernel<false>, grid, blk, 0, st, x, res, out, HW, eps, relu);
+  return scf_launch_status();
+}
+
+extern "C" int scf_instance_norm_ex(const float* x, float* res, float* out, int64_t planes, int HW, float eps,
+                                    int relu, int res_norm, scf_stream_t stream) {
+  if (!res_norm) return scf_instance_norm(x, res, out, planes, HW, eps, relu, stream);
+  if (!x || !res || !out || planes <= 0 || HW <= 0) return SCF_EINVAL;
+  if (planes > 0x7fffffffLL) return SCF_EUNSUPPORTED;
+  hipStream_t st = scf_stream(stream);
+  const dim3 grid((unsigned)planes), blk(256);
+  const bool vec = (HW % 4 == 0) && ((((uintptr_t)x | (uintptr_t)out | (uintptr_t)res) & 15) == 0);
+  const int n4 = HW / 4;
+  if (vec && n4 <= 256) scf_launch((instance_norm_kernel<1, 256, true>), grid, blk, 0, st, x, res, out, HW, eps, relu);
+  else if (vec && n4 <= 1024) scf_launch((instance_norm_kernel<4, 256, true>), grid, blk, 0, st, x, res, out, HW, eps, relu);
+  else if (vec && n4 <= 4096) scf_launch((instance_norm_kernel<16, 256, true>), grid, blk, 0, st, x, res, out, HW, eps, relu);
+  else if (vec && n4 <= 8192) scf_launch((instance_norm_kernel<8, 1024, true>), grid, dim3(1024), 0, st, x, res, out, HW, eps, relu);
+  else if (HW <= 32768) scf_launch(instance_norm_generic_kernel<true>, grid, blk, 0, st, x, res, out, HW, eps, relu);
+  else {
+    const int rc = scf_instance_norm(res, nullptr, res, planes, HW, eps, 0, stream);
+    return rc != SCF_OK ? rc : scf_instance_norm(x, res, out, planes, HW, eps, relu, stream);
+  }
   return scf_launch_status();
 }
 
diff --git a/scflow_amd/csrc/pose.hip b/scflow_amd/csrc/pose.hip
--- a/scflow_amd/csrc/pose.hip
+++ b/scflow_amd/csrc/pose.hip
@@ -12,13 +12,33 @@
 __device__ __forceinline__ void pose_store(const PoseOut& o, int n, float* __restrict__ d_rot, float* __restrict__ d_trans,
                                            float* R_out, float* t_out);
 
+typedef const __attribute__((address_space(3))) PoseMats* PoseMatsLds;
+__device__ __noinline__ float2 pose_flow_px(PoseMatsLds sp, int xi, int yi, float d, float invalid) {
+  const PoseMats& s = *(const PoseMats*)sp;
+  float u = invalid, v = invalid;
+  if (d > 0.f) {
+    const float x = (float)xi, y = (float)yi;
+    float X, Y, Z;
+    unproject(s, x, y, d, X, Y, Z);
+    const float px = s.R[0] * X + s.R[1] * Y + s.R[2] * Z + s.t[0];
+    const float py = s.R[3] * X + s.R[4] * Y + s.R[5] * Z + s.t[1];
+    const float pz = s.R[6] * X + s.R[7] * Y + s.R[8] * Z + s.t[2];
+    const float qx = s.K[0] * px + s.K[1] * py + s.K[2] * pz;
+    const float qy = s.K[3] * px + s.K[4] * py + s.K[5] * pz;
+    const float qz = s.K[6] * px + s.K[7] * py + s.K[8] * pz;
+    u = qx / qz - x;
+    v = qy / qz - y;
+  }
+  return make_float2(u, v);
+}
+
 __global__ __launch_bounds__(256) void reproject_flow_kernel(
     const float* __restrict__ depth, const float* __restrict__ K, const float* __restrict__ R0,
     const float* __restrict__ t0, const float* R, const float* t,
-    float* __restrict__ flow, int H, int W, float invalid, PoseUpdateArgs pu) {
+    float* __restrict__ flow, int H, int W, float invalid, int ngeo, PoseUpdateArgs pu) {
   __shared__ PoseMats s;
   __shared__ PoseOut po;
-  const int n = blockIdx.y;
+  const int n = blockIdx.y, ng = n % ngeo;
   const bool fused = pu.rot_all != nullptr;
   if (fused && threadIdx.x == 224) {
     PoseOut o;
@@ -26,47 +46,113 @@
     po = o;
     if (blockIdx.x == 0) pose_store(o, n, pu.d_rot, pu.d_trans, pu.R_out, pu.t_out);
   }
-  load_mats(&s, K, R0, t0, fused ? nullptr : R, fused ? nullptr : t, n);
-  if (fused) {
-    if (threadIdx.x < 9) s.R[threadIdx.x] = po.R[threadIdx.x];
-    if (threadIdx.x >= 64 && threadIdx.x < 67) s.t[threadIdx.x - 64] = po.t[threadIdx.x - 64];
-    __syncthreads();
-  }
+  load_mats(&s, K, R0, t0, nullptr, nullptr, ng);
+  if (threadIdx.x < 9) s.R[threadIdx.x] = fused ? po.R[threadIdx.x] : R[9 * n + threadIdx.x];
+  if (threadIdx.x >= 64 && threadIdx.x < 67) s.t[threadIdx.x - 64] = fused ? po.t[threadIdx.x - 64] : t[3 * n + threadIdx.x - 64];
+  __syncthreads();
   const int hw = H * W;
-  const float* dp = depth + (long long)n * hw;
+  const float* dp = depth + (long long)ng * hw;
   float* fx = flow + (long long)n * 2 * hw;
   float* fy = fx + hw;
+  const PoseMatsLds sp = (PoseMatsLds)&s;
   for (int idx = blockIdx.x * blockDim.x + threadIdx.x; idx < hw; idx += gridDim.x * blockDim.x) {
-    const float d = dp[idx];
-    float u = invalid, v = invalid;
-    if (d > 0.f) {
-      const int yi = idx / W, xi = idx - yi * W;
-      const float x = (float)xi, y = (float)yi;
-      float X, Y, Z;
-      unproject(s, x, y, d, X, Y, Z);
-      const float px = s.R[0] * X + s.R[1] * Y + s.R[2] * Z + s.t[0];
-      const float py = s.R[3] * X + s.R[4] * Y + s.R[5] * Z + s.t[1];
-      const float pz = s.R[6] * X + s.R[7] * Y + s.R[8] * Z + s.t[2];
-      const float qx = s.K[0] * px + s.K[1] * py + s.K[2] * pz;
-      const float qy = s.K[3] * px + s.K[4] * py + s.K[5] * pz;
-      const float qz = s.K[6] * px + s.K[7] * py + s.K[8] * pz;
-      u = qx / qz - x;
-      v = qy / qz - y;
-    }
-    fx[idx] = u;
-    fy[idx] = v;
+    const int yi = idx / W, xi = idx - yi * W;
+    const float2 f = pose_flow_px(sp, xi, yi, dp[idx], invalid);
+    fx[idx] = f.x;
+    fy[idx] = f.y;
   }
 }
 
 extern "C" int scf_reproject_flow(const float* depth, const float* K, const float* R0,
                                   const float* t0, const float* R, const float* t, float* flow,
                                   int N, int H, int W, float invalid_num, scf_stream_t stream) {
-  if (!depth || !K || !R0 || !t0 || !R || !t || !flow || N <= 0 || H <= 0 || W <= 0) return SCF_EINVAL;
-  if (N > 65535) return SCF_EUNSUPPORTED;
+  return scf_reproject_flow_iters(depth, K, R0, t0, R, t, flow, 1, N, H, W, invalid_num, stream);
+}
+
+int scf_reproject_flow_iters(const float* depth, const float* K, const float* R0, const float* t0, const float* R,
+                             const float* t, float* flow, int iters, int N, int H, int W, float invalid_num,
+                             scf_stream_t stream) {
+  if (!depth || !K || !R0 || !t0 || !R || !t || !flow || iters <= 0 || N <= 0 || H <= 0 || W <= 0) return SCF_EINVAL;
+  if ((int64_t)H * W > 0x7fffffffLL) return SCF_EINVAL;
+  if ((int64_t)iters * N > 65535) return SCF_EUNSUPPORTED;
   const int bx = (int)(scf_cdiv((int64_t)H * W, 256) < 64 ? scf_cdiv((int64_t)H * W, 256) : 64);
   const PoseUpdateArgs none = {};
-  scf_launch(reproject_flow_kernel, dim3(bx, N), dim3(256), 0, scf_stream(stream), depth, K,
-                     R0, t0, R, t, flow, H, W, invalid_num, none);
+  scf_launch(reproject_flow_kernel, dim3(bx, iters * N), dim3(256), 0, scf_stream(stream), depth, K,
+                     R0, t0, R, t, flow, H, W, invalid_num, N, none);
+  return scf_launch_status();
+}
+
+__global__ __launch_bounds__(256) void pose_update_flow_lr_kernel(
+    const float* __restrict__ depth, const float* __restrict__ K, const float* __restrict__ R0,
+    const float* __restrict__ t0, float* __restrict__ flow_lr, float* __restrict__ flow_copy, long long copy_nstride,
+    int H, int W, int h, int w, float sh, float sw, float mul, float invalid, PoseUpdateArgs pu) {
+#pragma clang fp contract(off)
+  __shared__ PoseMats s;
+  __shared__ PoseOut po;
+  const int n = blockIdx.y;
+  if (threadIdx.x == 224) {
+    PoseOut o;
+    pose_update_one(pu.rot_all, pu.trans_all, pu.label, pu.num_class, pu.label_mode, pu.R_in, pu.t_in, n, &o);
+    po = o;
+    if (blockIdx.x == 0) pose_store(o, n, pu.d_rot, pu.d_trans, pu.R_out, pu.t_out);
+  }
+  if (!flow_lr) return;
+  load_mats(&s, K, R0, t0, nullptr, nullptr, n);
+  if (threadIdx.x < 9) s.R[threadIdx.x] = po.R[threadIdx.x];
+  if (threadIdx.x >= 64 && threadIdx.x < 67) s.t[threadIdx.x - 64] = po.t[threadIdx.x - 64];
+  __syncthreads();
+  const float* dp = depth + (long long)n * H * W;
+  const PoseMatsLds sp = (PoseMatsLds)&s;
+  const int hw = h * w;
+  for (int idx = blockIdx.x * blockDim.x + threadIdx.x; idx < hw; idx += gridDim.x * blockDim.x) {
+    const int oy = idx / w, ox = idx - oy * w;
+    const float fy = sh * (float)oy;
+    int y0 = (int)fy;
+    if (y0 > H - 1) y0 = H - 1;
+    const int y1 = y0 + (y0 < H - 1 ? 1 : 0);
+    const float ly = fy - (float)y0, hy = 1.f - ly;
+    const float fx = sw * (float)ox;
+    int x0 = (int)fx;
+    if (x0 > W - 1) x0 = W - 1;
+    const int x1 = x0 + (x0 < W - 1 ? 1 : 0);
+    const float lx = fx - (float)x0, hx = 1.f - lx;
+    const float2 v00 = pose_flow_px(sp, x0, y0, dp[y0 * W + x0], invalid);
+    const float2 v01 = pose_flow_px(sp, x1, y0, dp[y0 * W + x1], invalid);
+    const float2 v10 = pose_flow_px(sp, x0, y1, dp[y1 * W + x0], invalid);
+    const float2 v11 = pose_flow_px(sp, x1, y1, dp[y1 * W + x1], invalid);
+    const float u = mul * (hy * (hx * v00.x + lx * v01.x) + ly * (hx * v10.x + lx * v11.x));
+    const float v = mul * (hy * (hx * v00.y + lx * v01.y) + ly * (hx * v10.y + lx * v11.y));
+    float* o = flow_lr + (long long)n * 2 * hw + idx;
+    o[0] = u;
+    o[hw] = v;
+    if (flow_copy) {
+      float* o2 = flow_copy + (long long)n * copy_nstride + idx;
+      o2[0] = u;
+      o2[hw] = v;
+    }
+  }
+}
+
+extern "C" int scf_pose_update_flow_lr(const float* rot_all, const float* trans_all, const int64_t* label, int num_class,
+                                       int label_mode, const float* R_in, const float* t_in, float* d_rot, float* d_trans,
+                                       float* R_out, float* t_out, const float* depth, const float* K, const float* R0,
+                                       const float* t0, float* flow_lr, float* flow_copy, int64_t flow_copy_nstride, int N,
+                                       int H, int W, int h, int w, float mul, float invalid_num, scf_stream_t stream) {
+  if (!rot_all || !trans_all || !label || !R_in || !t_in || !d_rot || !d_trans || !R_out || !t_out || num_class <= 0 ||
+      (label_mode & ~(SCF_POSE_LABEL_PER_SAMPLE | SCF_POSE_DEPTH_LINEAR)) || N <= 0)
+    return SCF_EINVAL;
+  if (flow_lr && (!depth || !K || !R0 || !t0 || H <= 0 || W <= 0 || h <= 0 || w <= 0 || (int64_t)H * W > 0x7fffffffLL))
+    return SCF_EINVAL;
+  if (flow_copy && !flow_lr) return SCF_EINVAL;
+  if (N > 65535) return SCF_EUNSUPPORTED;
+  const int bx = !flow_lr ? 1 : (int)(scf_cdiv((int64_t)h * w, 256) < 4 ? scf_cdiv((int64_t)h * w, 256) : 4);
+  if (bx > 1 && (R_in == R_out || t_in == t_out)) return SCF_EUNSUPPORTED;
+  const float sh = h > 1 ? (float)(H - 1) / (float)(h - 1) : 0.f;
+  const float sw = w > 1 ? (float)(W - 1) / (float)(w - 1) : 0.f;
+  const PoseUpdateArgs pu = {rot_all, trans_all, (const long long*)label, num_class, label_mode, R_in, t_in,
+                             d_rot, d_trans, R_out, t_out};
+  scf_launch(pose_update_flow_lr_kernel, dim3(bx, N), dim3(256), 0, scf_stream(stream), depth, K, R0, t0, flow_lr,
+             flow_copy, (long long)flow_copy_nstride, H, W, h, w, sh, sw, mul, invalid_num, pu);
   return scf_launch_status();
 }
 
@@ -86,7 +172,7 @@
   const PoseUpdateArgs pu = {rot_all, trans_all, (const long long*)label, num_class, label_mode, R_in, t_in,
                              d_rot, d_trans, R_out, t_out};
   scf_launch(reproject_flow_kernel, dim3(bx, N), dim3(256), 0, scf_stream(stream), depth, K,
-                     R0, t0, (const float*)nullptr, (const float*)nullptr, flow, H, W, invalid_num, pu);
+                     R0, t0, (const float*)nullptr, (const float*)nullptr, flow, H, W, invalid_num, N, pu);
   return scf_launch_status();
 }
 
diff --git a/scflow_amd/csrc/scf_common.h b/scflow_amd/csrc/scf_common.h
--- a/scflow_amd/csrc/scf_common.h
+++ b/scflow_amd/csrc/scf_common.h
@@ -118,3 +118,6 @@
                               int label_mode, const float* R_in, const float* t_in, float* d_rot, float* d_trans,
                               float* R_out, float* t_out, const float* depth, const float* K, const float* R0,
                               const float* t0, float* flow, int N, int H, int W, float invalid_num, scf_stream_t stream);
+int scf_reproject_flow_iters(const float* depth, const float* K, const float* R0, const float* t0, const float* R,
+                             const float* t, float* flow, int iters, int N, int H, int W, float invalid_num,
+                             scf_stream_t stream);
diff --git a/scflow_amd/csrc/scflow_iter.hip b/scflow_amd/csrc/scflow_iter.hip
--- a/scflow_amd/csrc/scflow_iter.hip
+++ b/scflow_amd/csrc/scflow_iter.hip
@@ -42,18 +42,42 @@
 
 static std::atomic<int> g_iter_merge{1};
 int scf_iter_merge_set(int v) { return (v < 0 || v > 1) ? SCF_EINVAL : g_iter_merge.exchange(v); }
+static std::atomic<int> g_iter_defer{1};
+int scf_iter_defer_set(int v) { return (v < 0 || v > 1) ? SCF_EINVAL : g_iter_defer.exchange(v); }
+static bool iter_deferred() {
+  return g_iter_merge.load(std::memory_order_relaxed) != 0 && g_iter_defer.load(std::memory_order_relaxed) != 0;
+}
+
+extern "C" int scf_scflow_outputs(const float* depth, const float* K, const float* R0, const float* t0, const float* rots,
+                                  const float* transs, float* flows, const float* flow_lr, const float* d_flow,
+                                  const float* mask_lr, float* fpreds, float* masks, int iters, int N, int H, int W, int h,
+                                  int w, float invalid_flow_num, scf_stream_t stream) {
+  if (iters <= 0 || N <= 0 || H <= 0 || W <= 0 || h <= 0 || w <= 0) return SCF_EINVAL;
+  if ((masks && !fpreds) || (fpreds && !flow_lr) || (masks && !mask_lr)) return SCF_EINVAL;
+  if (!iter_deferred()) return SCF_OK;
+  if (flows)
+    SCF_TRY(scf_reproject_flow_iters(depth, K, R0, t0, rots, transs, flows, iters, N, H, W, invalid_flow_num, stream));
+  if (fpreds) {
+    const int64_t pl = (int64_t)iters * N;
+    SCF_TRY(scf_resize_bilinear_jobs(flow_lr, d_flow, fpreds, pl * 2, (float)H / (float)h, masks ? mask_lr : nullptr, nullptr,
+                                     masks, masks ? pl : 0, 1.0f, nullptr, 1, 0, h, w, H, W, stream));
+  }
+  return SCF_OK;
+}
 
 extern "C" int scf_scflow_iteration(const scf_scflow_iter* it, scf_stream_t stream) {
   if (!it) return SCF_EINVAL;
   const bool merge = g_iter_merge.load(std::memory_order_relaxed) != 0;
   if (it->struct_size != (int32_t)sizeof(scf_scflow_iter)) return SCF_EINVAL;
-  if (!it->flow_in || !it->flow_out || !it->flow_pred || !it->mask_up || !it->flow_lr || !it->corr ||
+  const bool defer = it->defer_outputs != 0 && iter_deferred();
+  if ((!it->flow_in && !(defer && it->flow_lr_ready)) || !it->flow_out || !it->flow_pred || !it->mask_up || !it->flow_lr || !it->corr ||
       !it->R_in || !it->t_in || !it->R_out || !it->t_out || !it->d_rot || !it->d_trans || !it->hx ||
       it->N <= 0 || it->H <= 0 || it->W <= 0 || it->h <= 0 || it->w <= 0 || it->npass <= 0 || it->npass > 2)
     return SCF_EINVAL;
   if ((it->mask_flow || it->mask_corr) && !it->mask_prev) return SCF_EINVAL;
   const bool pair_flow = it->overlap_flow == 2, pair_mask = it->overlap_mask == 2;
-  const bool any_overlap = it->overlap_flow == 1 || it->overlap_mask == 1 || it->overlap_up == 1;
+  const bool up_aside = it->overlap_up == 1 && !defer;
+  const bool any_overlap = it->overlap_flow == 1 || it->overlap_mask == 1 || up_aside;
   if (any_overlap && !it->side_stream) return SCF_EINVAL;
   hipStream_t mainq = scf_stream(stream), sideq = scf_stream(it->side_stream);
   IterEvents* Ep = any_overlap ? iter_events() : nullptr;
@@ -65,9 +89,10 @@
   const float scale = (float)it->H / (float)it->h;
 
   const bool dual = merge && !it->mask_flow && it->flow_copy_dst != nullptr;
-  SCF_TRY(scf_resize_bilinear_jobs(it->flow_in, nullptr, it->flow_lr, (int64_t)N * 2, 1.0f / scale, nullptr, nullptr, nullptr,
-                                   0, 1.0f, dual ? it->flow_copy_dst : nullptr, 2, it->hx_nstride, it->H, it->W, it->h,
-                                   it->w, stream));
+  if (!(defer && it->flow_lr_ready))
+    SCF_TRY(scf_resize_bilinear_jobs(it->flow_in, nullptr, it->flow_lr, (int64_t)N * 2, 1.0f / scale, nullptr, nullptr, nullptr,
+                                     0, 1.0f, dual ? it->flow_copy_dst : nullptr, 2, it->hx_nstride, it->H, it->W, it->h,
+                                     it->w, stream));
   const float* flow_enc = it->flow_lr;
   if (it->mask_flow) {
     if (!it->flow_masked) return SCF_EINVAL;
@@ -144,9 +169,9 @@
       if (!fork_to(sideq, mainq, E.ev[3])) return SCF_ELAUNCH;
     }
   }
-  {
-    scf_stream_t uq = it->overlap_up == 1 ? it->side_stream : stream;
-    if (it->overlap_up == 1) {
+  if (!defer) {
+    scf_stream_t uq = up_aside ? it->side_stream : stream;
+    if (up_aside) {
       if (!fork_to(mainq, sideq, E.ev[4])) return SCF_ELAUNCH;
       br.open = true;
     }
@@ -189,7 +214,12 @@
     SCF_TRY(scf_linear_pair(it->fc2_out, it->rot_w, it->rot_b, it->rot_all, it->rot_O, it->trans_w, it->trans_b,
                             it->trans_all, it->trans_O, N, it->fc2_O, SCF_ACT_NONE, stream));
   }
-  {
+  if (defer) {
+    SCF_TRY(scf_pose_update_flow_lr(it->rot_all, it->trans_all, it->label, it->num_class, it->label_mode, it->R_in, it->t_in,
+                                    it->d_rot, it->d_trans, it->R_out, it->t_out, it->depth, it->K, it->R0, it->t0,
+                                    it->flow_lr_next, it->flow_lr_next && dual ? it->flow_copy_dst : nullptr, it->hx_nstride, N,
+                                    it->H, it->W, it->h, it->w, 1.0f / scale, it->invalid_flow_num, stream));
+  } else {
     const int rf = !merge ? SCF_EUNSUPPORTED : scf_pose_update_reproject(it->rot_all, it->trans_all, it->label, it->num_class, it->label_mode, it->R_in,
                                              it->t_in, it->d_rot, it->d_trans, it->R_out, it->t_out, it->depth, it->K, it->R0,
                                              it->t0, it->flow_out, N, it->H, it->W, it->invalid_flow_num, stream);
@@ -202,7 +232,7 @@
       SCF_TRY(rf);
     }
   }
-  if (it->overlap_up == 1) {
+  if (up_aside) {
     br.open = false;
     if (!fork_to(sideq, mainq, E.ev[5])) return SCF_ELAUNCH;
   }
diff --git a/scflow_amd/modules.py b/scflow_amd/modules.py
--- a/scflow_amd/modules.py
+++ b/scflow_amd/modules.py
@@ -133,6 +133,8 @@
             self.downsample = nn.Sequential(nn.Conv2d(inplanes, planes, 1, stride=stride, bias=True),
                                             mk(planes))
 
+    fuse_shortcut_norm = True
+
     def _bn(self, m):
         return (m.weight, m.bias, m.running_mean, m.running_var) if self.kind == 'BN' else None
 
@@ -160,6 +162,8 @@
         y2 = ops.conv2d(p['c2'], y)
         if 'ds' in p:
             idt = ops.conv2d(p['ds'], x)
+            if self.fuse_shortcut_norm:
+                return ops.instance_norm(y2, res=idt, relu=True, out=y2, res_norm=True)
             ops.instance_norm(idt, out=idt)
         else:
             idt = x
@@ -239,13 +243,16 @@
             qf, qc = bf.packed, bc.packed
             tf_, tc_ = ops.conv2d_pair((qf['c1'], yf), (qc['c1'], yc, dict(act=ACT_RELU)))
             ops.instance_norm(tf_, relu=True, out=tf_)
+            raw = False
             if 'ds' in qf:
                 if_, ic_ = ops.conv2d_pair((qf['ds'], yf), (qc['ds'], yc))
-                ops.instance_norm(if_, out=if_)
+                raw = bf.fuse_shortcut_norm
+                if not raw:
+                    ops.instance_norm(if_, out=if_)
             else:
                 if_, ic_ = yf, yc
             uf_, yc = ops.conv2d_pair((qf['c2'], tf_), (qc['c2'], tc_, dict(res=ic_, act=ACT_RELU)))
-            yf = ops.instance_norm(uf_, res=if_, relu=True, out=uf_)
+            yf = ops.instance_norm(uf_, res=if_, relu=True, out=uf_, res_norm=raw)
     return ops.conv2d_pair((pf['head'], yf), (pc['head'], yc, dict(out=out_c, act=head_act, act2=head_act2,
                                                                   act_split=head_split)))
 
@@ -622,10 +629,10 @@
     E = lambda *shape: torch.empty(shape, **f32)
     enc, ph = self.encoder, self.pose_pred
     kch = self.num_levels * (2 * self.radius + 1) ** 2
-    flow_lr, flow_m, corr = E(n, 2, h, w), (E(n, 2, h, w) if self.mask_flow else None), E(n, kch, h, w)
+    flow_lr, flow_m, corr = E(iters, n, 2, h, w), (E(n, 2, h, w) if self.mask_flow else None), E(n, kch, h, w)
     f1, c1, cf = E(n, 128, h, w), E(n, 256, h, w), E(n, 256, h, w)
     zbuf, heads, dm = E(2, n, hc, h, w), E(n, 512, h, w), E(n, 96, h, w)
-    d_flow, mask, m1, d1 = E(n, 2, h, w), E(n, 1, h, w), E(n, 64, h, w), E(n, 128, h, w)
+    d_flow, mask, m1, d1 = E(iters, n, 2, h, w), E(iters, n, 1, h, w), E(n, 64, h, w), E(n, 128, h, w)
     ones = ops.constant((n, 1, h, w), 1.0, depth.device) if (self.mask_flow or self.mask_corr) else None
     hv, xm = hx[:, :hc], hx[:, hc + cc:]
     flows, fpreds, masks = E(iters, n, 2, H, W), E(iters, n, 2, H, W), E(iters, n, 1, H, W)
@@ -636,12 +643,12 @@
     it.L, it.radius, it.tiled_levels, it.corr_channels = len(pyramid), self.radius, int(tiled), kch
     for l, lv in enumerate(pyramid):
         it.levels[l] = lv.data_ptr()
-    it.flow_lr, it.corr = flow_lr.data_ptr(), corr.data_ptr()
+    it.flow_lr, it.corr = flow_lr[0].data_ptr(), corr.data_ptr()
     it.mask_flow, it.mask_corr = int(self.mask_flow), int(self.mask_corr)
     it.flow_masked = None if flow_m is None else flow_m.data_ptr()
     keep = [pyramid, flow_lr, flow_m, corr, f1, c1, cf, zbuf, heads, dm, d_flow, mask, m1, d1, ones, hx, ctx]
     cd = lambda blk, *a, **k: ops.conv_desc(blk.packed, *a, act=blk.act, **k)[0]
-    it.flow0 = cd(enc.flow_net[0], flow_lr, out=f1)
+    it.flow0 = cd(enc.flow_net[0], flow_lr[0], out=f1)
     it.flow1 = cd(enc.flow_net[1], f1, out=cf[:, 192:])
     it.corr0 = cd(enc.corr_net[0], corr, out=c1)
     it.corr1 = cd(enc.corr_net[1], c1, out=cf[:, :192])
@@ -662,11 +669,11 @@
         it.gru[i] = arr[i]
     it.z, it.rh = zbuf[0].data_ptr(), zbuf[1].data_ptr()
     it.heads = ops.conv_desc(self.packed, hv, out=heads, act=ACT_RELU)[0]
-    it.fpred = ops.conv_desc(self.flow_pred.packed, heads[:, :256], out=d_flow)[0]
-    it.mpred = ops.conv_desc(self.mask_pred.packed, heads[:, 256:], out=mask, act=ACT_SIGMOID)[0]
-    it.menc0 = cd(self.mask_encoder[0], mask, out=m1)
+    it.fpred = ops.conv_desc(self.flow_pred.packed, heads[:, :256], out=d_flow[0])[0]
+    it.mpred = ops.conv_desc(self.mask_pred.packed, heads[:, 256:], out=mask[0], act=ACT_SIGMOID)[0]
+    it.menc0 = cd(self.mask_encoder[0], mask[0], out=m1)
     it.menc1 = cd(self.mask_encoder[1], m1, out=dm[:, 64:])
-    it.denc0 = cd(self.delta_flow_encoder[0], d_flow, out=d1)
+    it.denc0 = cd(self.delta_flow_encoder[0], d_flow[0], out=d1)
     it.denc1 = cd(self.delta_flow_encoder[1], d1, out=dm[:, :64])
     x0, x1 = hv, dm
     for i, blk in enumerate(ph.conv_layers):
@@ -706,15 +713,22 @@
     it.side_stream = ops.side_stream_handle() if any(int(b) == 1 for b in overlap) else None
     outs = ([], [], [], [], [], [], [])
     flow, rot, trans = init_flow, rot0, trans0
+    it.defer_outputs = 1
     for i in range(iters):
         it.flow_in, it.R_in, it.t_in = flow.data_ptr(), rot.data_ptr(), trans.data_ptr()
-        it.mask_prev = None if ones is None else (ones if i == 0 else mask).data_ptr()
+        it.mask_prev = None if ones is None else (ones if i == 0 else mask[i - 1]).data_ptr()
+        it.flow_lr, it.flow_lr_ready = flow_lr[i].data_ptr(), int(i > 0)
+        it.flow_lr_next = flow_lr[i + 1].data_ptr() if i + 1 < iters else None
+        it.fpred.out = it.denc0.in0 = d_flow[i].data_ptr()
+        it.mpred.out = it.menc0.in0 = mask[i].data_ptr()
         flow, rot, trans = flows[i], rots[i], transs[i]
         it.flow_out, it.flow_pred, it.mask_up = flow.data_ptr(), fpreds[i].data_ptr(), masks[i].data_ptr()
         it.R_out, it.t_out, it.d_rot, it.d_trans = rot.data_ptr(), trans.data_ptr(), drots[i].data_ptr(), dtranss[i].data_ptr()
         ops.scflow_iteration(it)
         for lst, v in zip(outs, (flow, fpreds[i], rot, trans, masks[i], drots[i], dtranss[i])):
             lst.append(v)
+    ops.scflow_outputs(depth, internel_k, rot0, trans0, rots, transs, invalid_flow_num, flows, flow_lr=flow_lr, d_flow=d_flow,
+                       mask_lr=mask, fpreds=fpreds, masks=masks)
     if any(overlap):
         pass
     del keep
diff --git a/scflow_amd/ops.py b/scflow_amd/ops.py
--- a/scflow_amd/ops.py
+++ b/scflow_amd/ops.py
@@ -16,7 +16,7 @@
 
 __all__ = ['record_conv_kernels', 'PackedConv', 'conv_desc', 'gru_passes', 'scflow_iteration', 'side_stream_handle', 'pyramid_layout', 'untile_level', 'level_storage_shape', 'sepconv_gru', 'pack_conv_weight', 'pack_conv_weight_f16x3', 'set_conv_precision', 'set_conv_winograd', 'get_conv_winograd', 'pack_conv_weight_wino', 'pack_conv_weight_wino1d', 'pack_conv_weight_wino1d4',
            'get_conv_precision', 'set_conv_kslices', 'conv_kslices', 'conv_kslices_for', 'constant', 'clear_constants', 'register_conv_workspace', 'choose_kc', 'conv2d', 'conv2d_pair', 'corr_build', 'corr_lookup',
-           'instance_norm', 'group_norm_relu', 'linear', 'fc_splitk', 'fc_slices', 'pose_update', 'reproject_flow',
+           'instance_norm', 'group_norm_relu', 'linear', 'fc_splitk', 'fc_slices', 'pose_update', 'reproject_flow', 'pose_update_flow_lr', 'scflow_outputs',
            'flow_corr_2d3d', 'pnp_params', 'pnp_ransac', 'pnp',
            'unproject_depth', 'linear_pair', 'resize_bilinear', 'convex_upsample', 'avgpool2x2', 'copy_channels',
            'ACT_NONE', 'ACT_RELU', 'ACT_SIGMOID', 'ACT_TANH', 'CONV_PLAIN', 'CONV_GRU_ZR',
@@ -684,7 +684,7 @@
     return list(zip(_read_timers([e[0] for e in evs]), [e[1] for e in evs], [e[2] for e in evs]))
 
 
-TUNE_KEYS = {'wino_variant': 1, 'dma_force_ksplit': 2, 'dma_ksplit_groups': 3, 'wino1d4': 4, 'lookup_pipe': 5, 'lookup_store': 6, 'conv_autoslice': 7, 'iter_merge': 8, 'wino1d4_half': 9, 'conv_pair': 10}
+TUNE_KEYS = {'wino_variant': 1, 'dma_force_ksplit': 2, 'dma_ksplit_groups': 3, 'wino1d4': 4, 'lookup_pipe': 5, 'lookup_store': 6, 'conv_autoslice': 7, 'iter_merge': 8, 'wino1d4_half': 9, 'conv_pair': 10, 'iter_defer': 11}
 
 
 def tune(key: str, value: int) -> int:
@@ -918,11 +918,17 @@
 
 
 def instance_norm(x: Tensor, res: Optional[Tensor] = None, relu: bool = False,
-                  out: Optional[Tensor] = None, eps: float = 1e-5) -> Tensor:
+                  out: Optional[Tensor] = None, eps: float = 1e-5, res_norm: bool = False) -> Tensor:
     px = _dense(x, 'x')
     n, c, h, w = x.shape
     if out is None:
         out = torch.empty_like(x)
+    if res_norm:
+        if res is None or res.shape != x.shape:
+            raise _lib.ScflowHipError('instance_norm(res_norm=True) needs a residual of the shape of x')
+        _lib.check(_lib.load().scf_instance_norm_ex(px, _dense(res, 'res'), _dense(out, 'out'), n * c, h * w, eps,
+                                                    int(relu), 1, _stream()), 'scf_instance_norm_ex')
+        return out
     _lib.check(_lib.load().scf_instance_norm(px, _opt(res, 'res'), _dense(out, 'out'), n * c,
                                              h * w, eps, int(relu), _stream()),
                'scf_instance_norm')
@@ -1037,6 +1043,64 @@
         _dense(rot, 'rot'), _dense(trans, 'trans'), _dense(out, 'out'), n, h, w,
         float(invalid_num), _stream()), 'scf_reproject_flow')
     return out
+
+
+def pose_update_flow_lr(rot_all: Tensor, trans_all: Tensor, label: Tensor, num_class: int, rot: Tensor, trans: Tensor,
+                        depth: Tensor, k: Tensor, rot0: Tensor, trans0: Tensor, size: Tuple[int, int], mul: float,
+                        invalid_num: float = 0., label_mode: int = 0, copy_dst: Optional[Tensor] = None):
+    n, H, W = depth.shape
+    h, w = size
+    if not label.is_cuda or label.dtype != torch.int64 or not label.is_contiguous():
+        raise _lib.ScflowHipError('label must be a contiguous int64 GPU tensor')
+    f32 = dict(dtype=torch.float32, device=depth.device)
+    d_rot, d_trans = torch.empty((n, 6), **f32), torch.empty((n, 3), **f32)
+    r_out, t_out = torch.empty((n, 3, 3), **f32), torch.empty((n, 3), **f32)
+    flow_lr = torch.empty((n, 2, h, w), **f32)
+    cp, cps = None, 0
+    if copy_dst is not None:
+        _dev(copy_dst, 'copy_dst')
+        if tuple(copy_dst.shape) != (n, 2, h, w) or copy_dst.stride()[1:] != (h * w, w, 1):
+            raise _lib.ScflowHipError('pose_update_flow_lr: copy_dst must be an (N, 2, h, w) view with dense planes')
+        cp, cps = copy_dst.data_ptr(), copy_dst.stride(0)
+    _lib.check(_lib.load().scf_pose_update_flow_lr(
+        _dense(rot_all, 'rot_all'), _dense(trans_all, 'trans_all'), label.data_ptr(), num_class, label_mode,
+        _dense(rot, 'rot'), _dense(trans, 'trans'), d_rot.data_ptr(), d_trans.data_ptr(), r_out.data_ptr(), t_out.data_ptr(),
+        _dense(depth, 'depth'), _dense(k, 'k'), _dense(rot0, 'rot0'), _dense(trans0, 'trans0'), flow_lr.data_ptr(), cp, cps,
+        n, H, W, h, w, float(mul), float(invalid_num), _stream()), 'scf_pose_update_flow_lr')
+    return d_rot, d_trans, r_out, t_out, flow_lr
+
+
+def scflow_outputs(depth: Optional[Tensor] = None, k: Optional[Tensor] = None, rot0: Optional[Tensor] = None,
+                   trans0: Optional[Tensor] = None, rots: Optional[Tensor] = None, transs: Optional[Tensor] = None,
+                   invalid_num: float = 0., flows: Optional[Tensor] = None, *, flow_lr: Optional[Tensor] = None,
+                   d_flow: Optional[Tensor] = None, mask_lr: Optional[Tensor] = None, size: Optional[Tuple[int, int]] = None,
+                   fpreds: Optional[Tensor] = None, masks: Optional[Tensor] = None):
+    P = lambda t, name: None if t is None else _dense(t, name)
+    ref = rots if rots is not None else flow_lr
+    f32 = dict(dtype=torch.float32, device=ref.device)
+    iters, n = ref.shape[:2]
+    H = W = h = w = 1
+    if rots is not None:
+        _, H, W = depth.shape
+        h, w = H, W
+        if flows is None:
+            flows = torch.empty((iters, n, 2, H, W), **f32)
+    if flow_lr is not None:
+        h, w = flow_lr.shape[-2:]
+        if rots is None:
+            H, W = size
+        elif size is not None and tuple(size) != (H, W):
+            raise _lib.ScflowHipError('scflow_outputs: size differs from the depth maps')
+        if fpreds is None:
+            fpreds = torch.empty((iters, n, 2, H, W), **f32)
+        if mask_lr is not None and masks is None:
+            masks = torch.empty((iters, n, 1, H, W), **f32)
+    _lib.check(_lib.load().scf_scflow_outputs(
+        P(depth, 'depth'), P(k, 'k'), P(rot0, 'rot0'), P(trans0, 'trans0'), P(rots, 'rots'), P(transs, 'transs'),
+        P(flows if rots is not None else None, 'flows'), P(flow_lr, 'flow_lr'), P(d_flow, 'd_flow'),
+        P(mask_lr if flow_lr is not None else None, 'mask_lr'), P(fpreds, 'fpreds'), P(masks, 'masks'), iters, n, H, W, h, w,
+        float(invalid_num), _stream()), 'scf_scflow_outputs')
+    return flows, fpreds, masks
 
 
 def filter_flow_by_mask_(flow: Tensor, mask: Tensor, invalid_num: float = 400.,
```

Result: no change. 2321 (median of 6 runs) (+0.4%).
